# simplerr/rust-renderer

Measured on AMD Instinct MI355X. Metric: Mrays/s (path rays: primary + bounce + sun-shadow + light-shadow) at 1920x1080, 20 spp = 20 frames x 1 spp; camera and sun at rest, the one-off builds of the camera grid and the sun grid outside the timed region (value_with_grid_builds charges them to these frames, value_tree_walk uses neither grid), higher is better.
Workload: dtype f32

## Files before the change

### rust-renderer_amd/csrc/context.hip

```cpp
#include <hip/hip_runtime.h>
#include <rccl/rccl.h>
#include <dlfcn.h>

#include <algorithm>
#include <atomic>
#include <chrono>
#include <cstdlib>
#include <cmath>
#include <cstdio>
#include <cstring>
#include <string>
#include <thread>
#include <vector>

#include "bvh.h"
#include "context_internal.h"
#include "device_scan.h"
#include "device_types.h"
#include "utopian_hip.h"

using namespace uh;

namespace {

std::string g_create_error;

struct HostMesh {
   std::vector<UhVertex> vertices;
   std::vector<uint32_t> indices;
   UhGpuMaterial material;
   float o2w[12];
   float w2o[9];
};

struct EventPair {
   hipEvent_t start, stop;
   int kind;
};

template <typename T>
struct DevBuf {
   T* p = nullptr;
   void* base = nullptr;
   size_t n = 0;
   hipError_t alloc(size_t count, size_t stagger_bytes = 0) {
      release();
      n = count;
      if (count == 0) return hipSuccess;
      hipError_t e = hipMalloc(&base, count * sizeof(T) + stagger_bytes);
      if (e == hipSuccess) p = reinterpret_cast<T*>(static_cast<char*>(base) + stagger_bytes);
      return e;
   }
   void release() {
      if (base) (void)hipFree(base);
      p = nullptr;
      base = nullptr;
      n = 0;
   }
};

struct SceneBins {
   DevBuf<uint32_t> tile_count, tile_cursor, rec_count, tri_mesh, chunks, entries;
   DevBuf<unsigned long long> totals;
   DevBuf<uint4> records;
   DevBuf<float> mats;
   std::vector<float> mats_host;
   uint64_t geom = 0;
   template <class F> void each(F&& f) {
      f(tile_count, 0), f(tile_cursor, 0), f(rec_count, 0), f(tri_mesh, 0), f(chunks, 0), f(entries, 0), f(totals, 0), f(records, 0), f(mats, 0);
   }
};

}

enum HybridStage : int {
   kStShadows, kStGbuffer, kStReflections, kStSsao, kStDeferred, kStSky, kStPresent, kHybridPasses,
   kStEnvCube = kHybridPasses, kStEnvIrradiance, kStEnvSpecular, kStEnvLut, kStShadowMaps, kStMarchingCubes, kHybridStages
};

constexpr uint32_t kMaxSlots = 8;
struct Slot {
   hipStream_t stream = nullptr;
   hipStream_t side = nullptr;
   hipEvent_t ev_traced = nullptr, ev_missed = nullptr, ev_shaded = nullptr, ev_shadowed = nullptr, ev_side_done = nullptr;
   hipEvent_t ev_acc = nullptr;
   hipEvent_t frame_start = nullptr, frame_stop = nullptr;
   DevBuf<float4> rec, radf, pixcol;
   DevBuf<uint32_t> queues[5];
   DevBuf<Control> control;
   PathState ps{};
   bool ready = false;
   size_t capacity = 0;

   hipError_t create(size_t n) {
      capacity = n;
      uint32_t shard_cap = 0;
      {
         const uint32_t runs = (uint32_t)((n + 63) / 64);
         uint32_t per_shard[kShards] = {0};
         for (uint32_t r = 0; r < runs; r++) per_shard[shard_of_run(r)]++;
         for (uint32_t s = 0; s < kShards; s++) shard_cap = per_shard[s] * 64 > shard_cap ? per_shard[s] * 64 : shard_cap;
      }
      hipError_t e;
#define SLOT_TRY(expr)                 \
   if ((e = (expr)) != hipSuccess) return e
      SLOT_TRY(hipStreamCreateWithFlags(&stream, hipStreamNonBlocking));
      SLOT_TRY(hipStreamCreateWithFlags(&side, hipStreamNonBlocking));
      for (hipEvent_t* ev : {&ev_traced, &ev_missed, &ev_shaded, &ev_shadowed, &ev_side_done, &ev_acc}) SLOT_TRY(hipEventCreateWithFlags(ev, hipEventDisableTiming));
      SLOT_TRY(hipEventCreate(&frame_start));
      SLOT_TRY(hipEventCreate(&frame_stop));
      const size_t stagger = 4352;
      const size_t cap_q = (size_t)shard_cap * kShards;
      const size_t plane = (n > cap_q ? n : cap_q) + stagger / sizeof(float4);
      SLOT_TRY(rec.alloc(plane * (2 * kRecQuads + 1), 0 * stagger));
      SLOT_TRY(radf.alloc(n, 1 * stagger));
      SLOT_TRY(pixcol.alloc(n, 2 * stagger));
      for (int qi = 0; qi < 5; qi++) SLOT_TRY(queues[qi].alloc((size_t)shard_cap * kShards * (qi == 4 ? 2 : 1)));
      SLOT_TRY(control.alloc(1));
      SLOT_TRY(hipMemsetAsync(control.p, 0, sizeof(Control), stream));
      SLOT_TRY(hipStreamSynchronize(stream));
#undef SLOT_TRY
      ps.set[0] = PathRecs{rec.p, plane};
      ps.set[1] = PathRecs{rec.p + plane * kRecQuads, plane};
      ps.hit = rec.p + plane * 2 * kRecQuads;
      ps.radf = radf.p;
      ps.pixcol = pixcol.p;
      for (int i = 0; i < 5; i++) ps.queue[i] = queues[i].p;
      ps.shard_cap = shard_cap;
      ready = true;
      return hipSuccess;
   }
   void destroy() {
      if (stream) (void)hipStreamSynchronize(stream);
      if (side) (void)hipStreamSynchronize(side);
      rec.release();
      radf.release();
      pixcol.release();
      for (auto& q : queues) q.release();
      control.release();
      for (hipEvent_t* ev : {&ev_traced, &ev_missed, &ev_shaded, &ev_shadowed, &ev_side_done, &ev_acc, &frame_start, &frame_stop}) {
         if (*ev) (void)hipEventDestroy(*ev);
         *ev = nullptr;
      }
      if (side) (void)hipStreamDestroy(side);
      if (stream) (void)hipStreamDestroy(stream);
      stream = side = nullptr;
      ready = false;
   }
};

constexpr uint32_t kRestirBatch = 16;
constexpr int kSpatialRing = 2 * (int)kRestirBatch + 1;

struct uh_ctx {
   int device = 0;
   Slot slots[kMaxSlots];
   uint32_t frames_in_flight = 4;
   uint32_t batch_frames = 0;
   uint32_t next_slot = 0;
   uint32_t shard_cap = 0;
   hipEvent_t last_acc = nullptr;
   hipStream_t restir_stream = nullptr;
   hipEvent_t ev_restir = nullptr, rs_start = nullptr, rs_stop = nullptr;
   bool restir_recorded = false;
   int spatial_cur = 0;
   hipEvent_t spatial_reader[kSpatialRing] = {};
   uint32_t rp_rank = 0, rp_world = 1, rp_band_rows = 0;
   size_t res_stride = 0;
   UhRestirExchangeFn rp_exchange = nullptr;
   void* rp_user = nullptr;
   hipEvent_t ev_band[kSpatialRing] = {};
   void* rccl = nullptr;
   hipEvent_t t_start = nullptr, t_stop = nullptr;
   Slot* last_slot = nullptr;
   hipStream_t& stream = slots[0].stream;
   PathState& ps = slots[0].ps;
   DevBuf<Control>& control = slots[0].control;
   bool overlap_miss = true, overlap_shadow = true;
   uint32_t W = 0, H = 0;
   uint32_t num_cus = 256;
   uint32_t closest_blocks_per_cu = 5, shadow_blocks_per_cu = 5;
   uint32_t cam_walk_whole = 512;
   bool fused_bounces = true;
   bool fused_always = false;
   static constexpr uint32_t kFusedMaxPaths = 4u << 20;
   uint32_t fused_blocks_per_cu = 4;
   static constexpr uint32_t kSingleFrameBlocksPerCu = 4;
   std::string err;

   std::vector<HostMesh> meshes;
   std::vector<UhGpuLight> lights;
   struct HostTex {
      uint32_t w, h;
      uchar4* dev;
      uint32_t tiles_x;
   };
   std::vector<HostTex> textures;
   bool built = false;

   DevBuf<float4> d_nodes, d_tris, d_shade, d_lights;
   DevBuf<MeshShade> d_meshes;
   DevBuf<float> d_obj_corners, d_world_corners, d_node_box;
   DevBuf<RefitMesh> d_refit_meshes;
   std::vector<uint32_t> packet_keys;
   std::vector<uint32_t> level_start;
   bool topology_valid = false;
   bool device_build = false, src_valid = false;
   uint32_t device_build_kind = 1;
   uint32_t ploc_sah_top = 1024;
   static constexpr uint32_t kPlocRadius = 8;
   DevBuf<float> d_src_corners;
   DevBuf<uint32_t> d_src_keys;
   DevBuf<float4> d_src_shade;
   float refit_ms = 0.0f;
   DevBuf<TexInfo> d_tex;
   DevBuf<float> d_lut;
   SceneDev scene{};

   DevBuf<float4> accumulation, gbuffer;
   DevBuf<uchar4> output;
   DevBuf<UhReservoir> reservoirs[3], spatial_ring;
   DevBuf<float4> gb_ray_o, gb_ray_d, gb_hit;
   DevBuf<DeviceStats> dstats;
   Images im{};

   bool count_visits = false, time_kernels = false, full_frame_restir = false;
   bool iso_reference = true;
   uint32_t shadow_map_size = 4096;
   bool furnace = false;
   uint64_t frames = 0;
   float build_ms = 0.0f, last_frame_ms = 0.0f;
   float ms_by_kind[5] = {0, 0, 0, 0, 0};
   uint32_t trace_closest_launches = 0, trace_light_launches = 0;
   bool frame_timed = false;
   std::vector<EventPair> pending, free_events;
   uint32_t bvh_nodes = 0, bvh_tris = 0;

   bool sun_grid_enabled = true;
   bool sun_valid = false;
   bool sun_attempted = false;
   bool sun_have_pending = false;
   uint64_t geom_version = 1, sun_geom = 0, sun_geom_pending = 0;
   float sun_dir_built[3] = {0, 0, 0}, sun_dir_pending[3] = {0, 0, 0};
   DevBuf<uint32_t> d_sun_cells;
   DevBuf<SunGridEntry> d_sun_entries;
   DevBuf<float4> d_sun_recs;
   DevBuf<float> d_sun_coarse;
   uint32_t sun_coarse_shift = 2;
   int64_t sun_inline_max_mb = -1;
   SunGridDev sun_dev{};
   SunGridLimits sun_limits;
   std::string sun_why;
   float sun_build_ms = 0.0f, sun_mean_list = 0.0f;
   float sun_fallback_area = 1.0f;
   uint32_t sun_cells = 0, sun_entries = 0, sun_max_list = 0;
   bool sun_this_frame = false;
   bool primary_implicit = true;
   bool sun_device_build = true;

   bool cam_grid_enabled = true;
   bool cam_valid = false, cam_attempted = false, cam_have_pending = false;
   uint64_t cam_geom = 0, cam_geom_pending = 0;
   float cam_mats[32] = {0}, cam_mats_pending[32] = {0};
   DevBuf<uint32_t> d_cam_cells;
   DevBuf<SunGridEntry> d_cam_entries;
   SunGridDev cam_dev{};
   SunGridLimits cam_limits;
   std::string cam_why;
   float cam_build_ms = 0.0f, cam_mean_list = 0.0f;
   uint32_t cam_cells = 0, cam_entries = 0, cam_max_list = 0, cam_max_list_interior = 0;
   bool cam_this_frame = false;

   uint32_t tp_rank = 0, tp_world = 1, tp_tile = 64;
   DevBuf<uint32_t> owned_pixels;
   uint32_t n_owned = 0;
   DevBuf<float4> tile_send, tile_recv;
   hipEvent_t ev_compose = nullptr;

   struct Hybrid {
      DevBuf<float4> pos, nrm, pbr;
      DevBuf<uchar4> alb, refl;
      DevBuf<uint8_t> shadow;
      DevBuf<uint32_t> queue, counter;
      DevBuf<HybridMesh> meshes;
      DevBuf<UhVertex> vertices;
      DevBuf<uint32_t> indices;
      uint64_t geom = 0;
      hipEvent_t waits[2 * kMaxSlots + 1] = {};
      struct Stage {
         hipEvent_t begin = nullptr, end = nullptr;
         bool ran = false, timed = false;
         float ms = 0.0f;
      } stage[kHybridStages];
      DevBuf<uint16_t> ssao;
      DevBuf<float4> deferred;
      DevBuf<uchar4> present;
      DevBuf<uint32_t> sky_counter;
      DevBuf<UhGpuLight> raw_lights;
      DevBuf<HybridLight> lights;
      size_t lights_uploaded = SIZE_MAX;
      uint32_t frame_lights = 0;
      DevBuf<float4> env, irr, spec;
      DevBuf<uint32_t> lut;
      DevBuf<float4> taps;
      uint32_t env_builds = 0;
      float env_sun[3] = {0, 0, 0}, env_eye[3] = {0, 0, 0};
      DevBuf<float> smaps;
      DevBuf<uint32_t> s_tile_count, s_tile_cursor, s_rec_count, s_tri_mesh, s_chunks, s_entries;
      DevBuf<unsigned long long> s_totals;
      DevBuf<uint4> s_records;
      DevBuf<float> s_mats;
      DevBuf<UhShadowmapParams> s_params;
      std::vector<float> s_mats_host;
      uint64_t s_geom = 0;
      bool params_set = false;
      UhShadowmapParams params{}, snapshot{}, pending{};
      uint32_t s_renders = 0, smap_size = 0, s_tris[4] = {0, 0, 0, 0};
      bool gbuffer_done = false;
      bool gbuffer_rasterised = false;
      DevBuf<float> gr_depth;
      DevBuf<uint32_t> gr_vis, gr_rec_of, gr_covered;
      SceneBins gr_bins;
      uint32_t gr_renders = 0, gr_pieces = 0;
      DevBuf<float> mc_depth;
      DevBuf<uint32_t> mc_vis, mc_rec_of, mc_covered;
      DevBuf<HybridLight> mc_lights;
      DevBuf<UhVertex> mc_verts;
      DevBuf<uint32_t> mc_block_counts, mc_tile_count, mc_tile_cursor, mc_rec_count, mc_chunks, mc_entries;
      DevBuf<unsigned long long> mc_totals;
      DevBuf<uint4> mc_records;
      DevBuf<float> mc_mats;
      DevBuf<HybridMesh> mc_mesh;
      uint32_t mc_renders = 0, mc_tris = 0, mc_pieces = 0, mc_lights_used = 0;
      float mc_time = 0.0f;

      template <class F> void rt_images(size_t n, F&& f) {
         f(pos, n), f(nrm, n), f(pbr, n), f(alb, n), f(refl, n), f(shadow, n), f(queue, n), f(counter, 1);
      }
      template <class F> void frame_images(size_t n, F&& f) {
         f(ssao, n), f(deferred, n), f(present, n), f(lights, UH_MAX_GPU_LIGHTS + 1), f(sky_counter, 1);
      }
      template <class F> void shadow_maps(F&& f) {
         f(smaps, 0), f(s_tile_count, 0), f(s_tile_cursor, 0), f(s_rec_count, 0), f(s_tri_mesh, 0), f(s_chunks, 0), f(s_entries, 0),
            f(s_totals, 0), f(s_records, 0), f(s_mats, 0), f(s_params, 0);
      }
      template <class F> void mc_images(size_t n, F&& f) {
         f(mc_depth, n), f(mc_vis, n), f(mc_rec_of, n), f(mc_lights, UH_MAX_GPU_LIGHTS + 1), f(mc_block_counts, kMcBlocks), f(mc_mats, 44),
            f(mc_mesh, 1), f(mc_totals, 3), f(mc_covered, 1);
      }
      template <class F> void mc_bins(F&& f) {
         f(mc_verts, 0), f(mc_tile_count, 0), f(mc_tile_cursor, 0), f(mc_rec_count, 0), f(mc_chunks, 0), f(mc_entries, 0), f(mc_records, 0);
      }
      template <class F> void gr_images(size_t n, F&& f) { f(gr_depth, n), f(gr_vis, n), f(gr_rec_of, n), f(gr_covered, 1); }
      template <class F> void env_maps(F&& f) {
         const size_t cube = env_mip_offset(kEnvMips);
         f(env, cube), f(irr, 6 * (size_t)kEnvSize * kEnvSize), f(spec, cube), f(lut, (size_t)kLutSize * kLutSize);
      }
   } hy;

   struct Forward {
      DevBuf<float4> color;
      DevBuf<float> depth;
      DevBuf<uint32_t> vis, rec_of, covered;
      DevBuf<uchar4> present;
      DevBuf<HybridLight> lights;
      SceneBins bins;
      uh_ctx::Hybrid::Stage stage[3];
      uint32_t renders = 0, pieces = 0, lights_used = 0;
      template <class F> void images(size_t n, F&& f) {
         f(depth, n), f(vis, n), f(rec_of, n), f(present, n), f(lights, UH_MAX_GPU_LIGHTS + 1), f(covered, 1), f(color, n);
      }
   } fw;
};

namespace {

int fail(uh_ctx* c, int code, const std::string& msg) {
   if (c)
      c->err = msg;
   else
      g_create_error = msg;
   return code;
}

#define HIP_TRY(ctx, expr)                                                                                   \
   do {                                                                                                      \
      hipError_t e_ = (expr);                                                                                \
      if (e_ != hipSuccess) return fail(ctx, e_ == hipErrorOutOfMemory ? UH_ERR_OUT_OF_MEMORY : UH_ERR_HIP, \
                                        std::string(#expr) + ": " + hipGetErrorString(e_));                 \
   } while (0)

// ... 835 lines not shown
      SunGridDev& d = c->sun_dev;
      std::memcpy(d.U, g.params.U, sizeof(d.U));
      std::memcpy(d.V, g.params.V, sizeof(d.V));
      std::memcpy(d.W, g.params.W, sizeof(d.W));
      d.u0 = g.params.u0;
      d.v0 = g.params.v0;
      d.inv_cell = g.params.inv_cell;
      d.nx = g.params.nx;
      d.ny = g.params.ny;
      d.max_walk = c->sun_limits.max_walk;
      d.cell_start = c->d_sun_cells.p;
      d.entries = c->d_sun_entries.p;
      c->sun_cells = g.params.nx * g.params.ny;
      c->sun_entries = (uint32_t)g.num_entries;
      c->sun_valid = true;
   }
   g.release();
   return attach_sun_inline_records(c);
}

static int attach_sun_inline_records(uh_ctx* c) {
   c->d_sun_recs.release();
   c->sun_dev.recs = nullptr;
   c->d_sun_coarse.release();
   c->sun_dev.coarse = nullptr;
   c->sun_dev.coarse_shift = c->sun_dev.coarse_nx = 0;
   if (c->sun_valid && c->sun_coarse_shift) {
      const uint32_t sh = c->sun_coarse_shift, b = 1u << sh, cnx = (c->sun_dev.nx + b - 1) / b, cny = (c->sun_dev.ny + b - 1) / b;
      HIP_TRY(c, c->d_sun_coarse.alloc((size_t)cnx * cny));
      HIP_TRY(c, (hipError_t)build_sun_coarse_cover((void*)c->stream, c->d_sun_cells.p, c->sun_dev.nx, c->sun_dev.ny, sh, c->d_sun_coarse.p));
      HIP_TRY(c, hipStreamSynchronize(c->stream));
      c->sun_dev.coarse = c->d_sun_coarse.p;
      c->sun_dev.coarse_shift = sh;
      c->sun_dev.coarse_nx = cnx;
   }
   const uint64_t n = c->sun_entries;
   const uint64_t budget = c->sun_inline_max_mb < 0 ? 4ull * 16 * kTriStride16 * c->scene.num_tris : (uint64_t)c->sun_inline_max_mb << 20;
   if (!c->sun_valid || n == 0 || n * 64ull > budget) return UH_OK;
   if (c->d_sun_recs.alloc((size_t)n * 4) != hipSuccess) {
      (void)hipGetLastError();
      return UH_OK;
   }
   HIP_TRY(c, (hipError_t)build_sun_inline_records((void*)c->stream, c->d_tris.p, c->d_sun_entries.p, n, c->d_sun_recs.p));
   HIP_TRY(c, hipStreamSynchronize(c->stream));
   c->sun_dev.recs = reinterpret_cast<const float*>(c->d_sun_recs.p);
   return UH_OK;
}

static int ensure_sun_grid(uh_ctx* c, const float dir[3]) {
   c->sun_this_frame = false;
   if (!c->sun_grid_enabled || c->scene.num_tris == 0) return UH_OK;
   const bool same_geom = c->sun_geom == c->geom_version;
   const bool same_dir = std::memcmp(dir, c->sun_dir_built, sizeof(float) * 3) == 0;
   if (same_geom && c->sun_attempted && same_dir) {
      c->sun_have_pending = false;
      c->sun_this_frame = c->sun_valid;
      return UH_OK;
   }
   if (c->sun_attempted) {
      const bool settled = c->sun_have_pending && c->sun_geom_pending == c->geom_version && std::memcmp(dir, c->sun_dir_pending, sizeof(float) * 3) == 0;
      std::memcpy(c->sun_dir_pending, dir, sizeof(float) * 3);
      c->sun_geom_pending = c->geom_version;
      c->sun_have_pending = true;
      if (!settled) return UH_OK;
   }
   const uint32_t n = c->scene.num_tris;
   if (c->sun_device_build) {
      if (int st = sync_all(c)) return st;
      const auto t0 = std::chrono::steady_clock::now();
      SunGridDevice g;
      const bool ok = build_sun_grid_device((void*)c->stream, c->d_tris.p, n, dir, c->sun_limits, nullptr, g);
      if (!ok && g.why_not.rfind("device build:", 0) == 0) return fail(c, UH_ERR_HIP, "sun grid: " + g.why_not);
      if (int st = adopt_sun_grid_device(c, g, ok, dir, c->geom_version)) return st;
      c->sun_build_ms = std::chrono::duration<float, std::milli>(std::chrono::steady_clock::now() - t0).count();
      c->sun_this_frame = c->sun_valid;
      return UH_OK;
   }
   int threads = (int)std::thread::hardware_concurrency();
   threads = threads < 1 ? 1 : (threads > 32 ? 32 : threads);
   if (int st = sync_all(c)) return st;
   const auto t0 = std::chrono::steady_clock::now();
   std::vector<float> packets(12 * (size_t)n);
   HIP_TRY(c, hipMemcpy2D(packets.data(), sizeof(TriPacket), c->d_tris.p, 16 * kTriStride16, sizeof(TriPacket), n, hipMemcpyDeviceToHost));
   SunGridHost g;
   const bool ok = build_sun_grid(packets.data(), n, dir, c->sun_limits, threads, g);
   if (int st = adopt_sun_grid(c, g, ok, dir, c->geom_version, 0.0f)) return st;
   c->sun_build_ms = std::chrono::duration<float, std::milli>(std::chrono::steady_clock::now() - t0).count();
   c->sun_this_frame = c->sun_valid;
   return UH_OK;
}

static int ensure_camera_grid(uh_ctx* c, const FrameParams& fp, uint32_t batch) {
   c->cam_this_frame = false;
   if (!c->cam_grid_enabled || c->scene.num_tris == 0) return UH_OK;
   float mats[32];
   std::memcpy(mats, fp.inv_view, sizeof(float) * 16);
   std::memcpy(mats + 16, fp.inv_proj, sizeof(float) * 16);
   const bool same = c->cam_attempted && c->cam_geom == c->geom_version && std::memcmp(mats, c->cam_mats, sizeof(mats)) == 0;
   if (same) {
      c->cam_have_pending = false;
      c->cam_this_frame = c->cam_valid;
      return UH_OK;
   }
   const bool settled = c->cam_have_pending && c->cam_geom_pending == c->geom_version && std::memcmp(mats, c->cam_mats_pending, sizeof(mats)) == 0;
   std::memcpy(c->cam_mats_pending, mats, sizeof(mats));
   c->cam_geom_pending = c->geom_version;
   c->cam_have_pending = true;
   if (!settled && batch < 8) return UH_OK;
   if (int st = sync_all(c)) return st;
   const auto t0 = std::chrono::steady_clock::now();
   SunGridDevice g;
   const bool ok = build_camera_grid_device((void*)c->stream, c->d_tris.p, c->scene.num_tris, fp.inv_view, fp.inv_proj, c->W, c->H, c->cam_limits, g);
   if (!ok && g.why_not.rfind("device build:", 0) == 0) return fail(c, UH_ERR_HIP, "camera grid: " + g.why_not);
   c->cam_attempted = true;
   c->cam_have_pending = false;
   c->cam_geom = c->geom_version;
   std::memcpy(c->cam_mats, mats, sizeof(mats));
   c->cam_valid = false;
   c->cam_why = g.why_not;
   c->cam_mean_list = (float)g.mean_list;
   c->cam_max_list = g.max_list;
   c->cam_max_list_interior = g.max_list_interior;
   c->cam_cells = c->cam_entries = 0;
   c->d_cam_cells.release();
   c->d_cam_entries.release();
   if (ok) {
      const size_t ncell = (size_t)g.params.nx * g.params.ny;
      c->d_cam_cells.p = g.cells;
      c->d_cam_cells.base = g.cells;
      c->d_cam_cells.n = ncell + 1;
      c->d_cam_entries.p = g.entries;
      c->d_cam_entries.base = g.entries;
      c->d_cam_entries.n = (size_t)g.num_entries;
      g.cells = nullptr;
      g.entries = nullptr;
      SunGridDev& d = c->cam_dev;
      d = SunGridDev{};
      d.nx = g.params.nx;
      d.ny = g.params.ny;
      d.max_walk = c->cam_limits.max_walk;
      d.walk_whole = c->cam_walk_whole;
      d.cell_start = c->d_cam_cells.p;
      d.entries = c->d_cam_entries.p;
      c->cam_cells = c->W * c->H;
      c->cam_entries = (uint32_t)g.num_entries;
      c->cam_valid = true;
   }
   g.release();
   c->cam_build_ms = std::chrono::duration<float, std::milli>(std::chrono::steady_clock::now() - t0).count();
   c->cam_this_frame = c->cam_valid;
   return UH_OK;
}

static int enqueue_path_trace(uh_ctx* c, Slot& s, const FrameParams& fp) {
   LaunchCfg lc = cfg(c);
   lc.stream = s.stream;
   if (fp.batch_frames == 1) {
      lc.closest_blocks_per_cu = std::min(lc.closest_blocks_per_cu, uh_ctx::kSingleFrameBlocksPerCu);
      lc.shadow_blocks_per_cu = std::min(lc.shadow_blocks_per_cu, uh_ctx::kSingleFrameBlocksPerCu);
   }
   Control* ctl = s.control.p;
   DeviceStats* st = c->dstats.p;
   for (uint32_t smp = 0; smp < fp.samples_per_frame; smp++) {
      HIP_TRY(c, hipMemsetAsync(ctl, 0, sizeof(Control), s.stream));
      uint32_t slot = 0;
      launch_generate(lc, fp, s.ps, ctl, smp);
      const bool gpu_idle = !c->last_acc || hipEventQuery(c->last_acc) == hipSuccess;
      const bool fused = c->fused_bounces && fp.batch_frames == 1 && fp.num_bounces >= 2 && fp.num_bounces <= 64 && s.ps.shard_cap < (1u << 23) &&
                         ((gpu_idle && fp.n_owned <= uh_ctx::kFusedMaxPaths) || c->fused_always);
      const bool fused_sun0 = fused && fp.sun_shadow_enabled == 1 && fp.lights_enabled != 1;
      for (uint32_t b = 0; b < (fused ? 1u : fp.num_bounces); b++) {
         begin_timed(c, (b == 0 && c->cam_this_frame) ? 3 : 0, s.stream);
         if (b == 0 && c->cam_this_frame) {
            launch_trace_camera_grid(lc, fp, c->scene, s.ps, ctl, st, slot, slot + 1, c->cam_dev, c->cam_max_list_interior > std::max(c->cam_dev.walk_whole, c->cam_dev.max_walk));
            slot += 2;
         } else
            launch_trace_closest(lc, c->scene, s.ps, ctl, st, b, slot++, b == 0 ? UH_RAY_PRIMARY : UH_RAY_BOUNCE);
         end_timed(c, s.stream);
         const bool side_shadow = c->overlap_shadow && (fp.sun_shadow_enabled == 1 || fp.lights_enabled == 1);
         const bool side_used = side_shadow || c->overlap_miss;
         if (side_used && b > 0) HIP_TRY(c, hipStreamWaitEvent(s.stream, s.ev_shadowed, 0));
         begin_timed(c, 2, s.stream);
         launch_shade_hit(lc, fp, c->scene, s.ps, c->im, ctl, st, b);
         if (!c->overlap_miss) launch_shade_miss(lc, fp, s.ps, ctl, st, b);
         end_timed(c, s.stream);
         LaunchCfg lsh = lc;
         hipStream_t sh_stream = s.stream;
         if (side_used) {
            HIP_TRY(c, hipEventRecord(s.ev_shaded, s.stream));
            HIP_TRY(c, hipStreamWaitEvent(s.side, s.ev_shaded, 0));
         }
         if (c->overlap_miss) {
            LaunchCfg ls = lc;
            ls.stream = s.side;
            begin_timed(c, 2, s.side);
            launch_shade_miss(ls, fp, s.ps, ctl, st, b);
            end_timed(c, s.side);
         }
         if (side_shadow) {
            lsh.stream = s.side;
            sh_stream = s.side;
         }
         if (fp.sun_shadow_enabled == 1 && !fused_sun0) {
            begin_timed(c, 1, sh_stream);
            if (c->sun_this_frame) {
               launch_trace_sun_grid(lsh, fp, c->scene, s.ps, ctl, st, b, slot++, c->sun_dev);
               launch_trace_shadow(lsh, fp, c->scene, s.ps, ctl, st, b, slot++, false, true);
            } else
               launch_trace_shadow(lsh, fp, c->scene, s.ps, ctl, st, b, slot++, false);
            end_timed(c, sh_stream);
         }
         if (fp.lights_enabled == 1) {
            begin_timed(c, 4, sh_stream);
            launch_trace_shadow(lsh, fp, c->scene, s.ps, ctl, st, b, slot++, true);
            end_timed(c, sh_stream);
         }
         if (side_used) HIP_TRY(c, hipEventRecord(s.ev_shadowed, s.side));
      }
      const bool join_side = (c->overlap_miss || c->overlap_shadow) && fp.num_bounces > 0;
      if (join_side && !fused_sun0) {
         HIP_TRY(c, hipEventRecord(s.ev_side_done, s.side));
         HIP_TRY(c, hipStreamWaitEvent(s.stream, s.ev_side_done, 0));
      }
      if (fused) {
         begin_timed(c, 0, s.stream);
         launch_path_fused(lc, fp, c->scene, s.ps, ctl, st, c->sun_dev, c->sun_this_frame, fused_sun0);
         end_timed(c, s.stream);
      }
      if (join_side && fused_sun0) {
         HIP_TRY(c, hipEventRecord(s.ev_side_done, s.side));
         HIP_TRY(c, hipStreamWaitEvent(s.stream, s.ev_side_done, 0));
      }
      if (fp.num_bounces > 0 && !fused) launch_flush_survivors(lc, fp, s.ps, ctl);
      const bool last = smp + 1 == fp.samples_per_frame;
      if (last && c->last_acc && c->last_acc != s.ev_acc) HIP_TRY(c, hipStreamWaitEvent(s.stream, c->last_acc, 0));
      launch_finish_sample(lc, fp, s.ps, c->im, smp, last);
   }
   if (fp.samples_per_frame == 0) {
      if (c->last_acc && c->last_acc != s.ev_acc) HIP_TRY(c, hipStreamWaitEvent(s.stream, c->last_acc, 0));
      launch_resolve(lc, c->im, c->W, c->H, fp.total_samples, fp.accumulation_limit);
   }
   HIP_TRY(c, hipEventRecord(s.ev_acc, s.stream));
   c->last_acc = s.ev_acc;
   return UH_OK;
}

struct uh_batch {
   FrameParams fp;
   uint32_t pass_mask = 0, batch = 0;
   bool restir_frame = false, reads_reservoirs = false;
   int read_slot[kMaxBatchFrames];
   LaunchCfg rc;
};

static UhReservoir* spatial_buf(uh_ctx* c, int slot) { return slot ? c->spatial_ring.p + (size_t)(slot - 1) * c->res_stride : c->reservoirs[2].p; }

static void restir_rows(const uh_ctx* c, UhRestirRows& r) {
   const uint32_t H = c->H, B = c->rp_world > 1 ? c->rp_band_rows : H;
   r = UhRestirRows{};
   r.rows_per_band = B;
   const uint32_t b0 = std::min<uint64_t>((uint64_t)c->rp_rank * B, H), b1 = std::min<uint64_t>((uint64_t)b0 + B, H);
   r.band_row0 = b0;
   r.band_rows = b1 - b0;
   if (b1 == b0) return;
   const uint32_t halo = 30;
   const uint32_t t0 = b0 > halo ? b0 - halo : 0, t1 = std::min<uint64_t>((uint64_t)b1 + halo, H);
   r.reuse_row0 = t0;
   r.reuse_rows = t1 - t0;
   if (b0 < halo && t1 < H) {
      r.reuse_extra_row0 = H - 1;
      r.reuse_extra_rows = 1;
   }
   const uint32_t g0 = t0 > 0 ? t0 - 1 : 0;
   r.cast_row0 = g0;
   r.cast_rows = t1 - g0;
   if (r.reuse_extra_rows) {
      const uint32_t e0 = std::max(H >= 2 ? H - 2 : 0u, t1);
      r.cast_extra_row0 = e0;
      r.cast_extra_rows = H - e0;
   }
}
static RowSpans spans_of(const uh_ctx* c, uint32_t row0, uint32_t rows, uint32_t extra0, uint32_t extra_rows) { return RowSpans{{row0, extra0}, {rows, extra_rows}, c->W}; }

static int batch_begin(uh_ctx* c, const UhViewUniformData* view, uint32_t pass_mask, uint32_t batch, uh_batch& bs) {
   if (!c) return UH_ERR_INVALID_ARGUMENT;
   if (!view) return fail(c, UH_ERR_INVALID_ARGUMENT, "uh_render_frame: null view");
   if (!c->built && c->topology_valid && view->rebuild_tlas == 1) {
      if (int st = uh_refit_acceleration(c)) return st;
   }
   if (!c->built) return fail(c, UH_ERR_NOT_BUILT, "uh_render_frame before uh_build_acceleration");
   if (view->num_bounces > kMaxBounces) return fail(c, UH_ERR_INVALID_ARGUMENT, "num_bounces > 64");
   if (view->samples_per_frame > 4096) return fail(c, UH_ERR_INVALID_ARGUMENT, "samples_per_frame > 4096 (the reference UI stops at 10)");
   if (view->num_lights > c->lights.size() && (view->lights_enabled == 1 || (pass_mask & UH_PASS_RESTIR)))
      return fail(c, UH_ERR_INVALID_ARGUMENT, "view.num_lights exceeds the lights added with uh_add_light");
   HIP_TRY(c, hipSetDevice(c->device));
   FrameParams& fp = bs.fp;
   fp = make_params(c, *view);
   fp.batch_frames = batch;
   for (uint32_t f = 0; f < batch; f++) {
      const uint32_t total = view->total_samples + f * view->samples_per_frame;
      fp.total_samples_of[f] = total;
      fp.frame_numbers[f] = (uint32_t)(int32_t)((float)total + view->time * 10000.0f);
   }
   c->cam_this_frame = false;
   const bool primary_rays = ((pass_mask & UH_PASS_REFERENCE_PT) && fp.num_bounces > 0 && fp.samples_per_frame > 0) || (pass_mask & UH_PASS_GBUFFER);
   if (primary_rays)
      if (int st = ensure_camera_grid(c, fp, batch)) return st;
   fp.primary_implicit = (c->primary_implicit && c->cam_this_frame && fp.samples_per_frame == 1) ? 1u : 0u;
   bs.pass_mask = pass_mask;
   bs.batch = batch;
   bs.restir_frame = (pass_mask & UH_PASS_RESTIR) != 0;
   bs.reads_reservoirs = (pass_mask & UH_PASS_REFERENCE_PT) && fp.lights_enabled == 1 && fp.use_ris == 1;

   if (batch > 1 && !(pass_mask & UH_PASS_REFERENCE_PT)) return fail(c, UH_ERR_INVALID_ARGUMENT, "uh_render_frames: a batch needs the path-tracing pass");
   if (batch > kRestirBatch && bs.restir_frame) return fail(c, UH_ERR_INVALID_ARGUMENT, "uh_render_frames: more reservoir-pass frames in one batch than the spatial ring holds");
   c->t_start = c->t_stop = nullptr;
   for (uint32_t f = 0; f < kMaxBatchFrames; f++) bs.read_slot[f] = c->spatial_cur;

   if (bs.restir_frame) {
      if (!c->restir_stream) {
         HIP_TRY(c, hipStreamCreateWithFlags(&c->restir_stream, hipStreamNonBlocking));
         HIP_TRY(c, hipEventCreateWithFlags(&c->ev_restir, hipEventDisableTiming));
         HIP_TRY(c, hipEventCreate(&c->rs_start));
// ... 292 lines not shown
      }
   }
   d_o.release();
   dd.release();
   dh.release();
   return UH_OK;
}

int uh_trace_any(uh_ctx* c, const float* rays, uint32_t n, uint8_t* out_occluded) {
   if (!c) return UH_ERR_INVALID_ARGUMENT;
   if (!c->built) return fail(c, UH_ERR_NOT_BUILT, "uh_trace_any before uh_build_acceleration");
   if (n == 0) return UH_OK;
   if (!rays || !out_occluded) return fail(c, UH_ERR_INVALID_ARGUMENT, "null argument");
   HIP_TRY(c, hipSetDevice(c->device));
   std::vector<float4> o(n), d(n);
   for (uint32_t i = 0; i < n; i++) {
      const float* r = rays + 8 * (size_t)i;
      o[i] = make_float4(r[0], r[1], r[2], r[3]);
      d[i] = make_float4(r[4], r[5], r[6], r[7]);
   }
   DevBuf<float4> d_o, dd;
   DevBuf<uint32_t> occ;
   HIP_TRY(c, d_o.alloc(n));
   HIP_TRY(c, dd.alloc(n));
   HIP_TRY(c, occ.alloc(n));
   HIP_TRY(c, hipMemcpyAsync(d_o.p, o.data(), n * sizeof(float4), hipMemcpyHostToDevice, c->stream));
   HIP_TRY(c, hipMemcpyAsync(dd.p, d.data(), n * sizeof(float4), hipMemcpyHostToDevice, c->stream));
   begin_timed(c, 1);
   launch_trace_any_raw(cfg(c), c->scene, d_o.p, dd.p, occ.p, n);
   end_timed(c);
   std::vector<uint32_t> h(n);
   if (int st = staged_read(c, h.data(), occ.p, n * sizeof(uint32_t))) return st;
   for (uint32_t i = 0; i < n; i++) out_occluded[i] = h[i] ? 1 : 0;
   d_o.release();
   dd.release();
   occ.release();
   return UH_OK;
}

int uh_get_stats(uh_ctx* c, UhStats* out) {
   if (!c || !out) return UH_ERR_INVALID_ARGUMENT;
   HIP_TRY(c, hipSetDevice(c->device));
   if (int st = sync_all(c)) return st;
   DeviceStats ds;
   if (int st = staged_read(c, &ds, c->dstats.p, sizeof(ds))) return st;
   drain_timed(c);
   if (c->frame_timed) {
      float ms = 0.0f;
      if (c->t_start && c->t_stop && hipEventElapsedTime(&ms, c->t_start, c->t_stop) == hipSuccess) c->last_frame_ms = ms;
   }
   std::memset(out, 0, sizeof(*out));
   for (int i = 0; i < UH_RAY_KINDS; i++) out->rays[i] = ds.rays[i];
   out->nodes_visited = ds.nodes_visited;
   out->tris_tested = ds.tris_tested;
   out->shadow_nodes_visited = ds.shadow_nodes_visited;
   out->shadow_tris_tested = ds.shadow_tris_tested;
   out->closest_hits = ds.closest_hits;
   out->misses = ds.misses;
   out->frames = c->frames;
   out->bvh_nodes = c->bvh_nodes;
   out->bvh_triangles = c->bvh_tris;
   out->build_ms = c->build_ms;
   out->last_frame_ms = c->last_frame_ms;
   out->trace_closest_ms = c->ms_by_kind[0];
   out->trace_shadow_ms = c->ms_by_kind[1];
   out->shade_ms = c->ms_by_kind[2];
   out->camera_grid_ms = c->ms_by_kind[3];
   out->trace_light_ms = c->ms_by_kind[4];
   out->trace_light_launches = c->trace_light_launches;
   out->light_nodes_visited = ds.light_nodes_visited;
   out->light_tris_tested = ds.light_tris_tested;
   out->trace_closest_launches = c->trace_closest_launches;
   out->sun_grid_cells = c->sun_valid ? c->sun_cells : 0;
   out->sun_grid_entries = c->sun_valid ? c->sun_entries : 0;
   out->sun_grid_build_ms = c->sun_build_ms;
   out->sun_grid_mean_list = c->sun_mean_list;
   out->sun_tree_rays = ds.sun_tree_rays;
   out->camera_grid_cells = c->cam_valid && c->cam_this_frame ? c->cam_cells : 0;
   out->camera_grid_entries = c->cam_valid && c->cam_this_frame ? c->cam_entries : 0;
   out->camera_grid_build_ms = c->cam_build_ms;
   out->camera_grid_mean_list = c->cam_mean_list;
   out->camera_tree_rays = ds.cam_tree_rays;
   out->camera_grid_tris_tested = ds.cam_tris_tested;
   out->sun_covered_rays = ds.sun_covered_rays;
   if (c->sun_valid) out->sun_grid_bytes = c->d_sun_cells.n * sizeof(uint32_t) + c->d_sun_entries.n * sizeof(SunGridEntry) + c->d_sun_recs.n * sizeof(float4) + c->d_sun_coarse.n * sizeof(float);
   if (c->cam_valid && c->cam_this_frame) out->camera_grid_bytes = c->d_cam_cells.n * sizeof(uint32_t) + c->d_cam_entries.n * sizeof(SunGridEntry);
   return UH_OK;
}

int uh_reset_stats(uh_ctx* c) {
   if (!c) return UH_ERR_INVALID_ARGUMENT;
   HIP_TRY(c, hipSetDevice(c->device));
   if (int st = sync_all(c)) return st;
   drain_timed(c);
   HIP_TRY(c, hipMemsetAsync(c->dstats.p, 0, sizeof(DeviceStats), c->stream));
   HIP_TRY(c, hipStreamSynchronize(c->stream));
   c->frames = 0;
   for (float& ms : c->ms_by_kind) ms = 0.0f;
   c->trace_closest_launches = c->trace_light_launches = 0;
   return UH_OK;
}

int uh_set_option(uh_ctx* c, const char* name, int value) {
   if (!c) return UH_ERR_INVALID_ARGUMENT;
   if (!name) return fail(c, UH_ERR_INVALID_ARGUMENT, "null option name");
   const std::string n(name);
   auto range = [&](int lo, int hi) { return value >= lo && value <= hi; };
   auto bad = [&](const char* what) { return fail(c, UH_ERR_INVALID_ARGUMENT, n + " " + what); };
   if (n == "count_visits")
      c->count_visits = value != 0;
   else if (n == "time_kernels") {
      if (c->time_kernels && !value) {
         (void)sync_all(c);
         drain_timed(c);
      }
      c->time_kernels = value != 0;
   }
   else if (n == "device_build") {
      if (!range(0, 2)) return bad("must be 0, 1 (PLOC) or 2 (radix tree)");
      if (c->device_build != (value != 0) || (value && c->device_build_kind != (uint32_t)value)) c->built = c->topology_valid = false;
      c->device_build = value != 0;
      if (value) c->device_build_kind = (uint32_t)value;
   } else if (n == "ploc_sah_top") {
      if (!range(0, 1 << 20)) return bad("must be 0..1048576");
      if (c->ploc_sah_top != (uint32_t)value && c->device_build) c->built = c->topology_valid = false;
      c->ploc_sah_top = (uint32_t)value;
   }
   else if (n == "sun_grid")
      c->sun_grid_enabled = value != 0;
   else if (n == "sun_grid_build") {
      c->sun_device_build = value != 0;
      c->sun_attempted = false;
   } else if (n == "sun_grid_density") {
      if (!range(1, 4096)) return bad("(entries per triangle) must be 1..4096");
      c->sun_limits.entries_per_triangle = (double)value;
      c->sun_attempted = false;
   } else if (n == "sun_grid_max_walk") {
      if (!range(1, 4096)) return bad("(longest list a ray tests itself) must be 1..4096");
      c->sun_limits.max_walk = (uint32_t)value;
      c->sun_attempted = false;
   } else if (n == "sun_grid_max_mb") {
      if (!range(1, 65536)) return bad("must be 1..65536");
      c->sun_limits.max_entries = ((uint64_t)value << 20) / sizeof(SunGridEntry);
      c->sun_attempted = false;
   } else if (n == "sun_grid_force") {
      const SunGridLimits defaults;
      c->sun_limits.max_mean_list = value ? 1e30 : defaults.max_mean_list;
      c->sun_limits.max_fallback_area = value ? 2.0 : defaults.max_fallback_area;
      c->sun_attempted = false;
   } else if (n == "sun_grid_inline_max_mb") {
      if (!range(-1, 1 << 20)) return bad("must be -1 (auto: 4 x the packet array), 0 (off) .. 1048576");
      c->sun_inline_max_mb = value;
      c->sun_attempted = false;
   } else if (n == "sun_grid_coarse") {
      if (!range(0, 6)) return bad("(log2 of the block edge in cells) must be 0..6");
      c->sun_coarse_shift = (uint32_t)value;
      c->sun_attempted = false;
   }
   else if (n == "camera_grid")
      c->cam_grid_enabled = value != 0;
   else if (n == "camera_grid_max_walk") {
      if (!range(1, 4096)) return bad("must be 1..4096");
      c->cam_limits.max_walk = (uint32_t)value;
      c->cam_attempted = false;
   } else if (n == "camera_grid_walk_whole") {
      if (!range(0, 65536)) return bad("must be 0..65536");
      c->cam_walk_whole = (uint32_t)value;
      c->cam_attempted = false;
   } else if (n == "camera_grid_max_mean_list_x10") {
      if (!range(1, 100000)) return bad("must be 1..100000");
      c->cam_limits.max_mean_list = value / 10.0;
      c->cam_attempted = false;
   } else if (n == "primary_implicit")
      c->primary_implicit = value != 0;
   else if (n == "full_frame_restir")
      c->full_frame_restir = value != 0;
   else if (n == "iso_reference_triangulation")
      c->iso_reference = value != 0;
   else if (n == "furnace")
      c->furnace = value != 0;
   else if (n == "shadow_map_size") {
      if (!range(16, 8192)) return bad("must be 16..8192");
      if ((uint32_t)value != c->shadow_map_size) {
         if (int st = sync_all(c)) return st;
         c->hy.shadow_maps([](auto& b, size_t) { b.release(); });
         c->hy.s_geom = 0;
         c->hy.smap_size = 0;
      }
      c->shadow_map_size = (uint32_t)value;
   }
   else if (n == "overlap")
      c->overlap_miss = c->overlap_shadow = value != 0;
   else if (n == "batch_frames") {
      if (!range(0, (int)kMaxBatchFrames)) return bad("must be 0 (auto) .. 32");
      c->batch_frames = (uint32_t)value;
   } else if (n == "frames_in_flight") {
      if (!range(1, (int)kMaxSlots)) return bad("must be 1..8");
      (void)sync_all(c);
      c->frames_in_flight = (uint32_t)value;
      c->next_slot = 0;
   } else if (n == "fused_bounces") {
      if (!range(-1, 8)) return bad("must be 0 (off), 1 (on when no frame is in flight), -1 (always on) or 2..8 (as 1, and blocks per CU of its grid)");
      c->fused_bounces = value != 0;
      c->fused_always = value == -1;
      if (value >= 2) c->fused_blocks_per_cu = (uint32_t)value;
   } else if (n == "trace_blocks_per_cu") {
      if (!range(1, 8)) return bad("must be 1..8");
      c->closest_blocks_per_cu = c->shadow_blocks_per_cu = (uint32_t)value;
   } else
      return fail(c, UH_ERR_INVALID_ARGUMENT, "unknown option: " + n);
   return UH_OK;
}

int uh_set_tile_partition(uh_ctx* c, uint32_t rank, uint32_t world, uint32_t tile_size) {
   if (!c) return UH_ERR_INVALID_ARGUMENT;
   if (world == 0 || rank >= world || tile_size == 0) return fail(c, UH_ERR_INVALID_ARGUMENT, "uh_set_tile_partition: need rank < world, tile_size > 0");
   HIP_TRY(c, hipSetDevice(c->device));
   if (int st = sync_all(c)) return st;
   c->tp_rank = rank;
   c->tp_world = world;
   c->tp_tile = tile_size;
   c->n_owned = c->W * c->H;
   c->owned_pixels.release();
   if (world > 1) {
      const uint32_t tiles_x = (c->W + tile_size - 1) / tile_size;
      std::vector<uint32_t> own;
      own.reserve((size_t)c->W * c->H / world + 1);
      for (uint32_t y = 0; y < c->H; y++)
         for (uint32_t x = 0; x < c->W; x++)
            if (((y / tile_size) * tiles_x + x / tile_size) % world == rank) own.push_back(y * c->W + x);
      c->n_owned = (uint32_t)own.size();
      HIP_TRY(c, c->owned_pixels.alloc(own.size() ? own.size() : 1));
      if (!own.empty()) HIP_TRY(c, hipMemcpy(c->owned_pixels.p, own.data(), own.size() * 4, hipMemcpyHostToDevice));
   }
   return UH_OK;
}

int uh_set_restir_partition(uh_ctx* c, uint32_t rank, uint32_t world, UhRestirExchangeFn exchange, void* user) {
   if (!c) return UH_ERR_INVALID_ARGUMENT;
   if (world == 0 || rank >= world) return fail(c, UH_ERR_INVALID_ARGUMENT, "uh_set_restir_partition: need rank < world");
   HIP_TRY(c, hipSetDevice(c->device));
   if (int st = sync_all(c)) return st;
   const size_t npix = (size_t)c->W * c->H;
   const uint32_t band_rows = (c->H + world - 1) / world;
   const size_t stride = std::max(npix, (size_t)band_rows * world * c->W);
   if (stride != c->res_stride) {
      DevBuf<UhReservoir> fresh;
      HIP_TRY(c, fresh.alloc(stride));
      HIP_TRY(c, hipMemsetAsync(fresh.p, 0, stride * sizeof(UhReservoir), c->stream));
      HIP_TRY(c, hipMemcpyAsync(fresh.p, c->im.reservoirs[2], npix * sizeof(UhReservoir), hipMemcpyDeviceToDevice, c->stream));
      HIP_TRY(c, hipStreamSynchronize(c->stream));
      c->reservoirs[2].release();
      c->reservoirs[2] = fresh;
      fresh.p = nullptr;
      fresh.n = 0;
      c->spatial_ring.release();
      c->res_stride = stride;
   } else if (c->spatial_cur != 0) {
      HIP_TRY(c, hipMemcpyAsync(c->reservoirs[2].p, c->im.reservoirs[2], npix * sizeof(UhReservoir), hipMemcpyDeviceToDevice, c->stream));
      HIP_TRY(c, hipStreamSynchronize(c->stream));
   }
   c->spatial_cur = 0;
   for (auto& r : c->spatial_reader) r = nullptr;
   c->im.reservoirs[2] = c->reservoirs[2].p;
   c->im.prev_spatial = c->reservoirs[2].p;
   c->rp_rank = rank;
   c->rp_world = world;
   c->rp_band_rows = world > 1 ? band_rows : c->H;
   c->rp_exchange = exchange;
   c->rp_user = user;
   return UH_OK;
}

int uh_get_restir_rows(uh_ctx* c, UhRestirRows* out) {
   if (!c || !out) return UH_ERR_INVALID_ARGUMENT;
   restir_rows(c, *out);
   return UH_OK;
}

namespace {
struct RcclApi {
   void* so = nullptr;
   decltype(&ncclGetUniqueId) GetUniqueId = nullptr;
   decltype(&ncclCommInitRank) CommInitRank = nullptr;
   decltype(&ncclCommDestroy) CommDestroy = nullptr;
   decltype(&ncclAllGather) AllGather = nullptr;
   decltype(&ncclSend) Send = nullptr;
   decltype(&ncclRecv) Recv = nullptr;
   decltype(&ncclGroupStart) GroupStart = nullptr;
   decltype(&ncclGroupEnd) GroupEnd = nullptr;
   decltype(&ncclCommCount) CommCount = nullptr;
   decltype(&ncclGetErrorString) GetErrorString = nullptr;
   std::string why;
};
RcclApi* rccl_api() {
   static RcclApi api;
   static bool tried = false;
   if (tried) return &api;
   tried = true;
   for (const char* name : {"librccl.so.1", "librccl.so", "/opt/rocm/lib/librccl.so.1"}) {
      api.so = dlopen(name, RTLD_NOW | RTLD_GLOBAL);
      if (api.so) break;
   }
   if (!api.so) {
      api.why = std::string("librccl not found: ") + (dlerror() ? dlerror() : "");
      return &api;
   }
// ... 1290 lines not shown
```

### rust-renderer_amd/csrc/device_types.h

```cpp
#pragma once
#include <hip/hip_runtime.h>

#include <cstdint>
#include <vector>

#include "bvh.h"
#include "sun_grid.h"
#include "utopian_hip.h"

namespace uh {

constexpr uint32_t kMaxBounces = 64;
constexpr uint32_t kQueueKinds = 5;
enum { Q_RAY = 0, Q_LIGHT = 1, Q_SUN_TREE = 2, Q_MISS = 3, Q_CAM_TREE = 4 };
constexpr uint32_t kLaunchSlots = kMaxBounces * 4 + 8;

constexpr uint32_t kShards = 32;
constexpr uint32_t kShardBits = 5;
static_assert((1u << kShardBits) == kShards, "kShards is a power of two");
__host__ __device__ inline uint32_t shard_of_run(uint32_t run) { return (run * 0x9E3779B1u) >> (32 - kShardBits); }

constexpr uint32_t kBounceStride = ((kMaxBounces + 1 + 31) / 32) * 32;
constexpr uint32_t kSlotStride = ((kLaunchSlots + 31) / 32) * 32;
struct Control {
   uint32_t q_count[kShards * kQueueKinds * kBounceStride];
   uint32_t cursor[kShards * kSlotStride];
};
__host__ __device__ inline uint32_t qc_index(uint32_t bounce, uint32_t kind, uint32_t shard) { return (shard * kQueueKinds + kind) * kBounceStride + bounce; }
__host__ __device__ inline uint32_t cursor_index(uint32_t slot, uint32_t shard) { return shard * kSlotStride + slot; }

struct DeviceStats {
   unsigned long long rays[UH_RAY_KINDS];
   unsigned long long nodes_visited, tris_tested, shadow_nodes_visited, shadow_tris_tested;
   unsigned long long closest_hits, misses;
   unsigned long long sun_tree_rays;
   unsigned long long cam_tree_rays;
   unsigned long long cam_tris_tested;
   unsigned long long sun_covered_rays;
   unsigned long long light_nodes_visited, light_tris_tested;
};

struct alignas(16) MeshShade {
   float w2o[9];
   uint32_t diffuse_map;
   float base_color[3];
   float type;
   float property;
   uint32_t pad;
   float metallic, roughness;
   float pad2[2];
};
static_assert(sizeof(MeshShade) == 80, "mesh shading record");

struct TexInfo {
   const uchar4* texels;
   uint32_t w, h;
   uint32_t tiles_x;
   uint32_t pad;
};

struct SceneDev {
   const uint4* nodes;
   const float4* tris;
   const float4* shade;
   const MeshShade* meshes;
   const TexInfo* textures;
   const float4* lights;
   const float* unorm_lut;
   uint32_t num_nodes, num_tris, num_meshes, num_textures, num_lights;
};

constexpr uint32_t kMaxBatchFrames = 32;

struct FrameParams {
   uint32_t batch_frames;
   uint32_t frame_numbers[kMaxBatchFrames];
   uint32_t total_samples_of[kMaxBatchFrames];
   const UhReservoir* spatial_of[kMaxBatchFrames];
   float inv_view[16], inv_proj[16], prev_pv[16];
   float sun_dir[3];
   uint32_t W, H, frame_number;
   uint32_t samples_per_frame, total_samples, num_bounces, accumulation_limit;
   uint32_t sky_enabled, sun_shadow_enabled, lights_enabled, use_ris, full_frame_restir;
   uint32_t primary_implicit;
   uint32_t furnace;
   uint32_t num_lights_used;
   uint32_t temporal_enabled, spatial_enabled;
   uint32_t tp_rank, tp_world, tp_tile, tiles_x;
   const uint32_t* owned_pixels;
   uint32_t n_owned;
};

constexpr uint32_t kRecQuads = 4;
enum { REC_ORIGIN = 0, REC_DIR = 1, REC_THR = 2, REC_RAD = 3 };
struct PathRecs {
   float4* base;
   size_t plane;
};
struct PathState {
   PathRecs set[2];
   float4* hit;
   float4* radf;
   float4* pixcol;
   uint32_t* queue[5];
   uint32_t shard_cap;
};
__host__ __device__ inline float4* rec_quad(const PathRecs& rec, uint32_t pos, int quad) { return rec.base + rec.plane * (size_t)quad + pos; }

struct RawRays {
   float4* ray_o;
   float4* ray_d;
   float4* hit;
};

struct Images {
   float4* accumulation;
   uchar4* output;
   float4* gbuffer_pos;
   UhReservoir* reservoirs[3];
   const UhReservoir* prev_spatial;
};

struct RowSpans {
   uint32_t row0[2], rows[2];
   uint32_t W;
   __host__ __device__ uint32_t total() const { return (rows[0] + rows[1]) * W; }
   __host__ __device__ uint32_t pixel_of(uint32_t j) const {
      const uint32_t first = rows[0] * W;
      return j < first ? row0[0] * W + j : row0[1] * W + (j - first);
   }
};
inline RowSpans whole_frame(uint32_t W, uint32_t H) { return RowSpans{{0, 0}, {H, 0}, W}; }

struct HybridMesh {
   float o2w[9];
   float w2o[9];
   uint32_t vertex_base, index_base;
   uint32_t diffuse_map, normal_map, metallic_roughness_map, occlusion_map;
};
struct HybridDev {
   float4* pos;
   float4* nrm;
   uchar4* alb;
   float4* pbr;
   uint8_t* shadow;
   uchar4* refl;
   uint32_t* queue;
   uint32_t* counter;
   const HybridMesh* meshes;
   const UhVertex* vertices;
   const uint32_t* indices;
   float sun_dir[3];
   float eye[3];
   uint32_t W, H, furnace;
};
struct HybridLight {
   float pos[3];
   float mode;
   float color[3];
   float spot;
   float att[3];
   float pad0;
   float dir[3];
   float pad1;
};
struct HybridFrameDev {
   uint16_t* ssao;
   float4* deferred;
   uchar4* present;
   uint32_t* sky_counter;
   HybridLight* lights;
   const UhGpuLight* raw_lights;
   float view[16], proj[16], inv_view[16];
   uint32_t num_lights;
   uint32_t ssao_on, rt_on, fxaa_on;
   float sun_raw[3];
};

struct LaunchCfg {
   hipStream_t stream;
   uint32_t num_cus;
   uint32_t closest_blocks_per_cu, shadow_blocks_per_cu;
   bool count_visits;
   uint32_t fused_blocks_per_cu = 4;
};

void launch_generate(const LaunchCfg&, const FrameParams&, const PathState&, Control*, uint32_t sample);
void launch_trace_closest(const LaunchCfg&, const SceneDev&, const PathState&, Control*, DeviceStats*, uint32_t bounce, uint32_t cursor_slot,
                          int ray_kind);
void launch_trace_camera_grid(const LaunchCfg&, const FrameParams&, const SceneDev&, const PathState&, Control*, DeviceStats*, uint32_t cursor_slot_grid, uint32_t cursor_slot_tree,
                              const SunGridDev&, bool leftovers_possible = true);
void launch_shade_miss(const LaunchCfg&, const FrameParams&, const PathState&, Control*, DeviceStats*, uint32_t bounce);
void launch_shade_hit(const LaunchCfg&, const FrameParams&, const SceneDev&, const PathState&, const Images&, Control*, DeviceStats*, uint32_t bounce);
void launch_flush_survivors(const LaunchCfg&, const FrameParams&, const PathState&, Control*);
void launch_path_fused(const LaunchCfg&, const FrameParams&, const SceneDev&, const PathState&, Control*, DeviceStats*, const SunGridDev& g, bool use_grid, bool sun_of_bounce0);
void launch_trace_shadow(const LaunchCfg&, const FrameParams&, const SceneDev&, const PathState&, Control*, DeviceStats*, uint32_t bounce,
                         uint32_t cursor_slot, bool light, bool sun_leftovers = false);
void launch_trace_sun_grid(const LaunchCfg&, const FrameParams&, const SceneDev&, const PathState&, Control*, DeviceStats*, uint32_t bounce,
                           uint32_t cursor_slot, const SunGridDev&);
void launch_finish_sample(const LaunchCfg&, const FrameParams&, const PathState&, const Images&, uint32_t sample, bool last);
void launch_resolve(const LaunchCfg&, const Images&, uint32_t W, uint32_t H, uint32_t total_samples, uint32_t limit);
void launch_gbuffer(const LaunchCfg&, const FrameParams&, const SceneDev&, const RawRays&, const Images&, DeviceStats*, const RowSpans& spans, uint32_t counted,
                    const SunGridDev* camera_grid = nullptr);
void launch_reset_reservoirs(const LaunchCfg&, const FrameParams&, const Images&, const RowSpans& spans);
void launch_initial_ris(const LaunchCfg&, const FrameParams&, const SceneDev&, const Images&, const RowSpans& spans);
void launch_temporal_reuse(const LaunchCfg&, const FrameParams&, const SceneDev&, const Images&, const RowSpans& spans);
void launch_spatial_reuse(const LaunchCfg&, const FrameParams&, const SceneDev&, const Images&, const RowSpans& spans);
void launch_trace_closest_raw(const LaunchCfg&, const SceneDev&, const float4* ray_o, const float4* ray_d, float4* hit, uint32_t n);
void launch_trace_any_raw(const LaunchCfg&, const SceneDev&, const float4* ray_o, const float4* ray_d, uint32_t* occluded, uint32_t n);
void launch_hybrid_clear(const LaunchCfg&, const HybridDev&);
void launch_hybrid_gbuffer(const LaunchCfg&, const FrameParams&, const SceneDev&, const HybridDev&, const SunGridDev* camera_grid);
void launch_hybrid_shadows(const LaunchCfg&, const SceneDev&, const HybridDev&);
void launch_hybrid_frame_clear(const LaunchCfg&, const HybridDev&, const HybridFrameDev&);
void launch_hybrid_ssao(const LaunchCfg&, const HybridDev&, const HybridFrameDev&);
void launch_hybrid_present(const LaunchCfg&, const HybridDev&, const HybridFrameDev&);
constexpr uint32_t kEnvSize = 512, kEnvMips = 8, kLutSize = 512;
constexpr uint32_t kIrrPhi = 252, kIrrTheta = 63;
__host__ __device__ inline uint32_t env_mip_offset(uint32_t m) {
   uint32_t o = 0;
   for (uint32_t k = 0; k < m; k++) o += 6u * (kEnvSize >> k) * (kEnvSize >> k);
   return o;
}
struct IblMaps {
   const float4* env;
   const float4* irr;
   const float4* spec;
   const uint32_t* lut;
};
struct EnvDev {
   float4* env;
   float4* irr;
   float4* spec;
   uint32_t* lut;
   const float4* taps;
   float eye[3];
   float sun[3];
};
void launch_env_cube(const LaunchCfg&, const EnvDev&);
void launch_env_irradiance(const LaunchCfg&, const EnvDev&);
void launch_env_specular(const LaunchCfg&, const EnvDev&);
void launch_env_brdf_lut(const LaunchCfg&, const EnvDev&);
void launch_hybrid_reflections(const LaunchCfg&, const SceneDev&, const HybridDev&, const IblMaps* ibl);
struct ShadowLookup {
   const float* maps;
   const UhShadowmapParams* params;
   uint32_t size;
};
void launch_hybrid_deferred(const LaunchCfg&, const SceneDev&, const HybridDev&, const HybridFrameDev&, const IblMaps* ibl,
                            const ShadowLookup* shadow);
constexpr uint32_t kShadowTile = 128;
struct ShadowDev {
   const UhVertex* vertices;
   const uint32_t* indices;
   const HybridMesh* meshes;
   const uint32_t* tri_mesh;
   const float* mats;
   uint32_t num_tris, num_meshes, size, tiles_x;
// ... 88 lines not shown
```

### rust-renderer_amd/csrc/kernels.hip

```cpp
#include <hip/hip_runtime.h>

#include <type_traits>

#include "device_math.h"
#include "device_types.h"
#include "hybrid_shading.h"
#include "ibl_device.h"

namespace uh {

constexpr int kBlock = 256;
constexpr int kWavesPerBlock = kBlock / 64;
constexpr int kSunRaysPerLane = 2;
constexpr int kShadeHitBlocks = 4;
constexpr int kLdsStack = 16;
constexpr int kSpillStack = (int)kTraversalStackEntries - kLdsStack;

struct Hit {
   float t, u, v;
   uint32_t idx;
   uint32_t key;
};

__device__ __forceinline__ float dot_fma(V3 a, V3 b) { return fmaf(a.z, b.z, fmaf(a.y, b.y, a.x * b.x)); }
// ... 257 lines not shown
         n = load_n;
         pool_base = load_base;
         loading = false;
      }
   }

   template <typename SrcFn>
   __device__ __forceinline__ void advance(const RaySource& src, RayPool<NA>& pool, SrcFn&& source_of) {
      const uint32_t lane = lane_id();
      if (q_n) {
         asm volatile("s_waitcnt lgkmcnt(0)" ::: "memory");
         if (lane < q_n) {
#pragma unroll
            for (int a = 0; a < NA; a++) dma16(source_of(a, q_id), pool.v[a]);
            pool.id[lane] = q_id;
         }
         load_n = q_n;
         load_base = q_base;
         loading = true;
         q_n = 0;
      }
      if (have_base) {
         const uint32_t b = __builtin_amdgcn_readfirstlane(r_base);
         have_base = false;
         if (b < src.count) {
            q_base = b;
            q_n = src.count - b < kPool ? src.count - b : kPool;
            if (lane < q_n) q_id = src.queue ? ld_stream(src.queue + b + lane) : b + lane;
         } else {
            drained = true;
         }
      }
      if (!drained) {
         if (src.cursor) {
            if (lane == 0) r_base = atomicAdd(src.cursor, kPool);
         } else {
            r_base = (static_k * src.num_waves + src.wave_index) * kPool;
            static_k++;
         }
         have_base = true;
      }
   }
};

constexpr int kRefill = 8;
template <int NA, typename SrcFn, typename TakeFn>
__device__ __forceinline__ bool refill_lanes(Feeder<NA>& f, const RaySource& src, RayPool<NA>& pool, bool lane_idle, SrcFn&& source_of, TakeFn&& take) {
   if (++f.iterations > (1u << 24)) return false;
   const unsigned long long idle = __ballot(lane_idle);
   if (idle == 0ull) return true;
   const uint32_t n_idle = (uint32_t)__popcll(idle);
   f.land();
   const uint32_t avail = f.n - f.pos;
   if (avail != 0 && (n_idle >= (uint32_t)kRefill || n_idle == 64u)) {
      const uint32_t prefix = __builtin_amdgcn_mbcnt_hi((uint32_t)(idle >> 32), __builtin_amdgcn_mbcnt_lo((uint32_t)idle, 0u));
      if (lane_idle && prefix < avail) take(f.pos + prefix);
      f.pos += n_idle < avail ? n_idle : avail;
   }
   if (f.pos >= f.n && !f.loading) {
      if (f.empty()) return n_idle != 64u || avail != 0;
      f.advance(src, pool, source_of);
   }
   return true;
}

template <bool ANY, bool COUNT, bool CAP = false>
__device__ __forceinline__ bool trav_step(const uint4* __restrict__ nodes, const float4* __restrict__ tris, Trav& t, uint32_t* lds_col, uint32_t* spill, bool& occluded,
                                          uint32_t& n_nodes, uint32_t& n_tris) {
   const bool at_node = !(t.cur & kLeafBit);
   const uint32_t packet = t.cur & ~kLeafBit;
   const uint4* rec = at_node ? nodes + kNodeStride16 * (size_t)packet : (const uint4*)tris + kTriStride16 * (size_t)packet;
   uint4 w0 = rec[0], w1 = rec[1], w2 = rec[2];
   asm volatile("" : "+v"(w2.z), "+v"(w2.w));
   bool pop;
   if (at_node) {
      if (COUNT) n_nodes++;
      pop = !node_compute<ANY, CAP>(w0, w1, w2, t, lds_col, spill);
   } else {
      if (COUNT) n_tris++;
      const float4 ta = make_float4(__uint_as_float(w0.x), __uint_as_float(w0.y), __uint_as_float(w0.z), __uint_as_float(w0.w));
      const float4 tb = make_float4(__uint_as_float(w1.x), __uint_as_float(w1.y), __uint_as_float(w1.z), __uint_as_float(w1.w));
      const float4 tc = make_float4(__uint_as_float(w2.x), __uint_as_float(w2.y), __uint_as_float(w2.z), __uint_as_float(w2.w));
      pop = true;
      if (tri_compute<ANY>(ta, tb, tc, packet, t.o, t.d, t.tmin, t.tlimit, t.best) && ANY) {
         occluded = true;
         t.cur = kEmptyRef;
         pop = false;
      }
   }
   if (pop) t.cur = trav_pop(t, lds_col, spill);
   return t.cur == kEmptyRef;
}

template <bool COUNT>
__global__ __launch_bounds__(kBlock, 6) void k_trace_closest(SceneDev sc, bool sharded, const float4* __restrict__ ray_o,
                                                               const float4* __restrict__ ray_d, float4* __restrict__ hit_out, uint32_t shard_cap, Control* ctl,
                                                               DeviceStats* stats, uint32_t bounce, uint32_t cursor_slot, int ray_kind, uint32_t raw_count,
                                                               const uint32_t* __restrict__ listed) {
   const bool range_in_w = !sharded;
   __shared__ uint32_t s_stack[kWavesPerBlock][kLdsStack][64];
   __shared__ RayPool<2> s_pool[kWavesPerBlock];
   const uint32_t lane = lane_id();
   const uint32_t wave = threadIdx.x >> 6;
   uint32_t* lds_col = &s_stack[wave][0][lane];
   RayPool<2>& pool = s_pool[wave];
   RaySource src;
   uint32_t seg = 0;
   if (sharded) {
      const ShardCtx sx = shard_ctx();
      seg = sx.shard * shard_cap;
      src.queue = listed ? listed + seg : nullptr;
      src.count = ctl->q_count[qc_index(bounce, listed ? Q_CAM_TREE : Q_RAY, sx.shard)];
      src.cursor = &ctl->cursor[cursor_index(cursor_slot, sx.shard)];
      src.wave_index = src.num_waves = 0;
      if (sx.lb == 0 && threadIdx.x == 0) {
         if (!listed) atomicAdd(&stats->rays[ray_kind], (unsigned long long)src.count);
         else if (src.count) atomicAdd(&stats->cam_tree_rays, (unsigned long long)src.count);
      }
   } else {
      src.queue = nullptr;
      src.count = raw_count;
      src.cursor = nullptr;
      src.wave_index = blockIdx.x * kWavesPerBlock + wave;
      src.num_waves = gridDim.x * kWavesPerBlock;
   }
   const uint4* __restrict__ nodes = sc.nodes;
   const float4* __restrict__ tris = sc.tris;
   auto source_of = [&](int a, uint32_t pos) { return (a == 0 ? ray_o : ray_d) + seg + pos; };
   Feeder<2> f;
   Trav t;
   t.cur = kEmptyRef;
   t.sp = 0;
   uint32_t where = 0, n_nodes = 0, n_tris = 0;
   uint32_t spill[kSpillStack];
   auto take = [&](uint32_t slot) {
      where = seg + (listed ? pool.id[slot] : f.pool_base + slot);
      const float4 ro = pool.v[0][slot], rd = pool.v[1][slot];
      trav_init(t, ro, rd, range_in_w ? ro.w : 0.001f, range_in_w ? rd.w : 10000.0f, INFINITY);
   };
   while (refill_lanes<2>(f, src, pool, t.cur == kEmptyRef, source_of, take)) {
      if (t.cur != kEmptyRef) {
         bool occluded = false;
         if (trav_step<false, COUNT>(nodes, tris, t, lds_col, spill, occluded, n_nodes, n_tris))
            st_rec(hit_out + where, make_float4(t.best.t, t.best.u, t.best.v, __uint_as_float(t.best.idx)));
      }
   }
   if (COUNT) {
      atomicAdd(&stats->nodes_visited, (unsigned long long)n_nodes);
      atomicAdd(&stats->tris_tested, (unsigned long long)n_tris);
   }
}

struct ShadowRay {
   float4 ro, rd, lit;
   float tlimit;
};
template <bool LIGHT>
__device__ __forceinline__ ShadowRay make_shadow_ray(const SceneDev& sc, const FrameParams& fp, float4 ro, float4 thr, float4 rad) {
   ShadowRay s;
   s.ro = make_float4(ro.x, ro.y, ro.z, 0.001f);
   s.tlimit = INFINITY;
   if (LIGHT) {
      const int light_index = (int)__float_as_uint(rad.w);
      V3 lpos = v3(0, 0, 0);
      if (light_index >= 0 && (uint32_t)light_index < sc.num_lights) lpos = xyz(sc.lights[2 * light_index]);
      const V3 o = v3(ro.x, ro.y, ro.z);
      const V3 dir = normalize3(lpos - o);
      s.tlimit = length3(lpos - o);
      const float f = thr.w;
      s.lit = make_float4(rad.x + thr.x * f, rad.y + thr.y * f, rad.z + thr.z * f, rad.w);
      s.rd = make_float4(dir.x, dir.y, dir.z, 10000.0f);
   } else {
      s.lit = make_float4(rad.x + thr.x, rad.y + thr.y, rad.z + thr.z, rad.w);
      s.rd = make_float4(fp.sun_dir[0], fp.sun_dir[1], fp.sun_dir[2], 10000.0f);
   }
   return s;
}

template <bool COUNT, bool LIGHT>
__global__ __launch_bounds__(kBlock, 5) void k_trace_shadow(SceneDev sc, FrameParams fp, PathState ps, Control* ctl, DeviceStats* stats, uint32_t bounce,
                                                              uint32_t cursor_slot, bool leftovers) {
   __shared__ uint32_t s_stack[kWavesPerBlock][kLdsStack][64];
   __shared__ RayPool<3> s_pool[kWavesPerBlock];
   const uint32_t lane = lane_id();
   const uint32_t wave = threadIdx.x >> 6;
   uint32_t* lds_col = &s_stack[wave][0][lane];
   RayPool<3>& pool = s_pool[wave];
   const ShardCtx sx = shard_ctx();
   const uint32_t seg = sx.shard * ps.shard_cap;
   RaySource src;
   src.queue = LIGHT ? ps.queue[2] + seg : leftovers ? ps.queue[3] + seg : nullptr;
   src.count = LIGHT ? ctl->q_count[qc_index(bounce, Q_LIGHT, sx.shard)] : leftovers ? ctl->q_count[qc_index(bounce, Q_SUN_TREE, sx.shard)] : ctl->q_count[qc_index(bounce + 1, Q_RAY, sx.shard)];
   src.cursor = &ctl->cursor[cursor_index(cursor_slot, sx.shard)];
   src.wave_index = src.num_waves = 0;
   if (sx.lb == 0 && threadIdx.x == 0) {
      if (!leftovers) atomicAdd(&stats->rays[LIGHT ? UH_RAY_LIGHT_SHADOW : UH_RAY_SUN_SHADOW], (unsigned long long)src.count);
      else if (src.count) atomicAdd(&stats->sun_tree_rays, (unsigned long long)src.count);
   }
   const uint4* __restrict__ nodes = sc.nodes;
   const float4* __restrict__ tris = sc.tris;
   const PathRecs rec = ps.set[(bounce + 1) & 1];
   float4* rad = rec_quad(rec, seg, REC_RAD);
   auto source_of = [&](int a, uint32_t pos) { return (const float4*)rec_quad(rec, seg + pos, a == 0 ? REC_ORIGIN : a == 1 ? REC_THR : REC_RAD); };
   Feeder<3> f;
   Trav t;
   t.cur = kEmptyRef;
   t.sp = 0;
   uint32_t id = 0, n_nodes = 0, n_tris = 0;
   float4 lit = make_float4(0.0f, 0.0f, 0.0f, 0.0f);
   uint32_t spill[kSpillStack];
   auto take = [&](uint32_t slot) {
      id = pool.id[slot];
      const ShadowRay s = make_shadow_ray<LIGHT>(sc, fp, pool.v[0][slot], pool.v[1][slot], pool.v[2][slot]);
      lit = s.lit;
      trav_init(t, s.ro, s.rd, s.ro.w, s.rd.w, s.tlimit);
   };
   while (refill_lanes<3>(f, src, pool, t.cur == kEmptyRef, source_of, take)) {
      if (t.cur != kEmptyRef) {
         bool occluded = false;
         if (trav_step<true, COUNT>(nodes, tris, t, lds_col, spill, occluded, n_nodes, n_tris) && !occluded) st_stream(rad + id, lit);
      }
   }
   if (COUNT) {
      atomicAdd(LIGHT ? &stats->light_nodes_visited : &stats->shadow_nodes_visited, (unsigned long long)n_nodes);
      atomicAdd(LIGHT ? &stats->light_tris_tested : &stats->shadow_tris_tested, (unsigned long long)n_tris);
   }
}

template <int N, int I = 0, typename F>
__device__ __forceinline__ void static_for(F&& f) {
   if constexpr (I < N) {
      f(std::integral_constant<int, I>{});
      static_for<N, I + 1>(f);
   }
}

__device__ __forceinline__ void sun_cell_of(const SunGridDev& g, float pu, float pv, uint32_t& cx, uint32_t& cy) {
   float fx = (pu - g.u0) * g.inv_cell, fy = (pv - g.v0) * g.inv_cell;
   fx = !(fx >= 0.0f) ? 0.0f : fx;
   fy = !(fy >= 0.0f) ? 0.0f : fy;
   const float max_x = (float)(g.nx - 1), max_y = (float)(g.ny - 1);
   fx = fx > max_x ? max_x : fx;
   fy = fy > max_y ? max_y : fy;
   cx = (uint32_t)fx;
   cy = (uint32_t)fy;
}
__device__ __forceinline__ bool sun_coarse_covered(float coarse, float pw) { return pw < coarse && coarse - pw < kSunCoarseReach; }

template <bool COUNT, bool INLINE>
__global__ __launch_bounds__(kBlock) void k_trace_sun_grid(SceneDev sc, FrameParams fp, PathState ps, Control* ctl, DeviceStats* stats, uint32_t bounce,
                                                            uint32_t cursor_slot, SunGridDev g) {
   const uint32_t lane = lane_id();
   const ShardCtx sx = shard_ctx();
   const uint32_t seg = sx.shard * ps.shard_cap;
   const PathRecs rec = ps.set[(bounce + 1) & 1];
   const uint32_t count = ctl->q_count[qc_index(bounce + 1, Q_RAY, sx.shard)];
   uint32_t* cursor = &ctl->cursor[cursor_index(cursor_slot, sx.shard)];
   const V3 d = v3(fp.sun_dir[0], fp.sun_dir[1], fp.sun_dir[2]);
   uint32_t n_tris = 0, n_covered = 0;
   uint32_t* q_tree = ps.queue[3] + seg;
   uint32_t* n_tree = &ctl->q_count[qc_index(bounce, Q_SUN_TREE, sx.shard)];
   constexpr int K = kSunRaysPerLane;
   typedef float f4_t __attribute__((ext_vector_type(4)));
   const f4_t* __restrict__ recs = reinterpret_cast<const f4_t*>(g.recs);
   const f4_t* __restrict__ tris = reinterpret_cast<const f4_t*>(sc.tris);
   const uint2* __restrict__ entries = reinterpret_cast<const uint2*>(g.entries);
   const uint4* __restrict__ cells = reinterpret_cast<const uint4*>(g.cell_start);
   for (;;) {
      uint32_t base = 0;
      if (lane == 0) base = atomicAdd(cursor, 64u * K);
      base = __builtin_amdgcn_readfirstlane(base);
      if (base >= count) break;
      uint32_t id[K];
      bool valid[K];
      static_for<K>([&](auto kc) {
         constexpr int k = decltype(kc)::value;
         id[k] = base + 64u * k + lane;
         valid[k] = id[k] < count;
      });
      float4 ro[K];
      static_for<K>([&](auto kc) {
         constexpr int k = decltype(kc)::value;
         ro[k] = valid[k] ? ld_rec(rec_quad(rec, seg + id[k], REC_ORIGIN)) : make_float4(0.0f, 0.0f, 0.0f, 0.0f);
      });
      float pw[K];
      uint32_t cx[K], cy[K];
      bool covered[K], ask[K];
      static_for<K>([&](auto kc) {
         constexpr int k = decltype(kc)::value;
         const V3 o = v3(ro[k].x, ro[k].y, ro[k].z);
         const float pu = dot_fma(v3(g.U[0], g.U[1], g.U[2]), o), pv = dot_fma(v3(g.V[0], g.V[1], g.V[2]), o);
         pw[k] = dot_fma(v3(g.W[0], g.W[1], g.W[2]), o);
         sun_cell_of(g, pu, pv, cx[k], cy[k]);
         covered[k] = false;
      });
      if (g.coarse) {
         float cw[K];
         static_for<K>([&](auto kc) {
            constexpr int k = decltype(kc)::value;
            cw[k] = valid[k] ? g.coarse[(cy[k] >> g.coarse_shift) * g.coarse_nx + (cx[k] >> g.coarse_shift)] : -INFINITY;
         });
         static_for<K>([&](auto kc) {
            constexpr int k = decltype(kc)::value;
            covered[k] = valid[k] && sun_coarse_covered(cw[k], pw[k]);
         });
      }
      uint4 cs[K];
      uint32_t end[K];
      static_for<K>([&](auto kc) {
         constexpr int k = decltype(kc)::value;
         ask[k] = valid[k] && !covered[k];
         cs[k] = make_uint4(0u, 0u, 0u, 0u);
         end[k] = 0u;
         if (ask[k]) {
            const uint32_t cell = cy[k] * g.nx + cx[k];
            cs[k] = cells[cell];
            end[k] = cells[cell + 1].x;
         }
      });
      bool defer[K], walk[K], lit[K];
      f4_t ra[K], rb[K], rc[K];
      uint2 en[K], nxt[K];
      static_for<K>([&](auto kc) {
         constexpr int k = decltype(kc)::value;
         const float cover = __uint_as_float(cs[k].y);
         const bool cov = ask[k] && pw[k] < cover && cover - pw[k] < kSunCoverReach;
         covered[k] = covered[k] || cov;
         defer[k] = ask[k] && !cov && (cx[k] == 0 || cy[k] == 0 || cx[k] + 1 == g.nx || cy[k] + 1 == g.ny || end[k] - cs[k].x > g.max_walk);
         walk[k] = ask[k] && !cov && !defer[k] && cs[k].x < end[k];
         lit[k] = ask[k] && !cov && !defer[k] && !walk[k];
         if (walk[k]) {
            if constexpr (INLINE) {
               const f4_t* r = recs + 4 * (size_t)cs[k].x;
               ra[k] = r[0];
               rb[k] = r[1];
               rc[k] = r[2];
            } else {
               en[k] = make_uint2(cs[k].z, cs[k].w);
               if (__uint_as_float(en[k].y) < pw[k]) {
                  walk[k] = false;
                  lit[k] = true;
               } else {
                  const f4_t* r = tris + kTriStride16 * (size_t)en[k].x;
                  ra[k] = r[0];
                  rb[k] = r[1];
                  rc[k] = r[2];
                  nxt[k] = cs[k].x + 1 < end[k] ? entries[cs[k].x + 1] : make_uint2(0u, 0u);
               }
            }
         }
         if (COUNT) n_covered += covered[k] ? 1u : 0u;
      });
      static_for<K>([&](auto kc) {
         constexpr int k = decltype(kc)::value;
         if (walk[k]) {
            const V3 o = v3(ro[k].x, ro[k].y, ro[k].z);
            Hit best;
            best.t = 10000.0f;
            best.u = best.v = 0.0f;
            best.idx = kEmptyRef;
            best.key = 0xffffffffu;
            uint32_t e = cs[k].x;
            float4 a = make_float4(ra[k].x, ra[k].y, ra[k].z, ra[k].w), b = make_float4(rb[k].x, rb[k].y, rb[k].z, rb[k].w), c = make_float4(rc[k].x, rc[k].y, rc[k].z, rc[k].w);
            bool occluded = false;
            if constexpr (INLINE) {
               const f4_t* r = recs + 4 * (size_t)e;
               for (;;) {
                  if (c.z < pw[k]) break;
                  if (COUNT) n_tris++;
                  if (tri_compute<true>(a, b, c, 0u, o, d, 0.001f, INFINITY, best)) {
                     occluded = true;
                     break;
                  }
                  e++;
                  if (e >= end[k] || c.w < pw[k]) break;
                  r += 4;
                  const f4_t na = r[0], nb = r[1], nc = r[2];
                  a = make_float4(na.x, na.y, na.z, na.w);
                  b = make_float4(nb.x, nb.y, nb.z, nb.w);
                  c = make_float4(nc.x, nc.y, nc.z, nc.w);
               }
            } else {
               uint2 cur = en[k], nx = nxt[k];
               for (;;) {
                  if (COUNT) n_tris++;
                  if (tri_compute<true>(a, b, c, cur.x, o, d, 0.001f, INFINITY, best)) {
                     occluded = true;
                     break;
                  }
                  e++;
                  if (e >= end[k] || __uint_as_float(nx.y) < pw[k]) break;
                  cur = nx;
                  if (e + 1 < end[k]) nx = entries[e + 1];
                  const f4_t* r = tris + kTriStride16 * (size_t)cur.x;
                  const f4_t na = r[0], nb = r[1], nc = r[2];
                  a = make_float4(na.x, na.y, na.z, na.w);
                  b = make_float4(nb.x, nb.y, nb.z, nb.w);
                  c = make_float4(nc.x, nc.y, nc.z, nc.w);
               }
            }
            lit[k] = !occluded;
         }
      });
      float4 thr[K], rad[K];
      static_for<K>([&](auto kc) {
         constexpr int k = decltype(kc)::value;
         if (lit[k]) {
            thr[k] = ld_rec(rec_quad(rec, seg + id[k], REC_THR));
            rad[k] = ld_rec(rec_quad(rec, seg + id[k], REC_RAD));
         }
      });
      static_for<K>([&](auto kc) {
         constexpr int k = decltype(kc)::value;
         if (lit[k]) st_rec(rec_quad(rec, seg + id[k], REC_RAD), make_float4(rad[k].x + thr[k].x, rad[k].y + thr[k].y, rad[k].z + thr[k].z, rad[k].w));
      });
      static_for<K>([&](auto kc) {
         constexpr int k = decltype(kc)::value;
         if (__ballot(defer[k]) != 0ull) {
            const uint32_t slot = wave_append(n_tree, defer[k]);
            if (defer[k]) st_stream(q_tree + slot, id[k]);
         }
      });
   }
   if (sx.lb == 0 && threadIdx.x == 0) {
      atomicAdd(&stats->rays[UH_RAY_SUN_SHADOW], (unsigned long long)count);
      if (COUNT) atomicAdd(&stats->shadow_nodes_visited, (unsigned long long)count);
   }
   if (COUNT) {
      atomicAdd(&stats->shadow_tris_tested, (unsigned long long)n_tris);
      atomicAdd(&stats->sun_covered_rays, (unsigned long long)n_covered);
   }
}

template <bool COUNT>
__global__ __launch_bounds__(kBlock) void k_trace_camera_grid(SceneDev sc, FrameParams fp, PathState ps, Control* ctl, DeviceStats* stats, uint32_t cursor_slot, SunGridDev g) {
   const uint32_t lane = lane_id();
   const ShardCtx sx = shard_ctx();
   const uint32_t seg = sx.shard * ps.shard_cap;
   const uint32_t* __restrict__ queue = ps.queue[0] + seg;
   const uint32_t count = ctl->q_count[qc_index(0, Q_RAY, sx.shard)];
   uint32_t* cursor = &ctl->cursor[cursor_index(cursor_slot, sx.shard)];
   const PathRecs rec = ps.set[0];
   const float4* __restrict__ tris = sc.tris;
   uint32_t* q_tree = ps.queue[3] + seg;
   uint32_t* n_tree = &ctl->q_count[qc_index(0, Q_CAM_TREE, sx.shard)];
   uint32_t n_tris = 0;
   for (;;) {
      const uint32_t base = next_batch(cursor);
      if (base >= count) break;
      const uint32_t i = base + lane;
      const bool valid = i < count;
      bool defer = false;
      if (valid) {
         const uint32_t id = ld_stream(queue + i);
         const uint32_t k = id % fp.n_owned;
         const uint32_t pix = fp.owned_pixels ? fp.owned_pixels[k] : k;
         const uint32_t px = pix % fp.W, py = pix / fp.W;
         const uint32_t cell = (py + 1) * g.nx + (px + 1);
         uint32_t e = g.cell_start[cell];
         const uint32_t end = g.cell_start[cell + 1];
         const bool sorted = end - e <= g.max_walk;
         defer = end - e > (g.walk_whole > g.max_walk ? g.walk_whole : g.max_walk);
         if (defer && fp.primary_implicit) {
            float4 ro, rd;
            primary_state(fp, id, ro, rd);
            st_rec(rec_quad(rec, seg + i, REC_ORIGIN), ro);
            st_rec(rec_quad(rec, seg + i, REC_DIR), rd);
         }
         if (!defer) {
            float4 ro, rd;
            if (fp.primary_implicit)
               primary_state(fp, id, ro, rd);
            else {
               ro = ld_rec(rec_quad(rec, seg + i, REC_ORIGIN));
               rd = ld_rec(rec_quad(rec, seg + i, REC_DIR));
            }
            const V3 o = v3(ro.x, ro.y, ro.z), d = v3(rd.x, rd.y, rd.z);
            Hit best;
            best.t = 10000.0f;
            best.u = best.v = 0.0f;
            best.idx = kEmptyRef;
            best.key = 0xffffffffu;
            uint2 en = make_uint2(0u, 0u);
            if (e < end) en = reinterpret_cast<const uint2*>(g.entries)[e];
            while (e < end) {
               if (sorted && -__uint_as_float(en.y) > best.t) break;
               const uint32_t pk = en.x;
               uint2 nxt = make_uint2(0u, 0u);
               if (e + 1 < end) nxt = reinterpret_cast<const uint2*>(g.entries)[e + 1];
               const float4 a = tris[kTriStride16 * (size_t)pk + 0], b = tris[kTriStride16 * (size_t)pk + 1], c = tris[kTriStride16 * (size_t)pk + 2];
               if (COUNT) n_tris++;
               tri_compute<false>(a, b, c, pk, o, d, 0.001f, INFINITY, best);
               en = nxt;
               e++;
            }
            st_rec(ps.hit + seg + i, make_float4(best.t, best.u, best.v, __uint_as_float(best.idx)));
         }
      }
      if (__ballot(defer) != 0ull) {
         const uint32_t slot = wave_append(n_tree, defer);
         if (defer) st_stream(q_tree + slot, i);
      }
   }
   if (sx.lb == 0 && threadIdx.x == 0) atomicAdd(&stats->rays[UH_RAY_PRIMARY], (unsigned long long)count);
   if (COUNT) atomicAdd(&stats->cam_tris_tested, (unsigned long long)n_tris);
}

__global__ __launch_bounds__(kBlock) void k_gbuffer_camera_grid(SceneDev sc, RawRays ps, RowSpans spans, uint32_t W, SunGridDev g) {
   const uint32_t n = spans.total();
   const float4* __restrict__ tris = sc.tris;
   for (uint32_t j = blockIdx.x * kBlock + threadIdx.x; j < n; j += gridDim.x * kBlock) {
      const uint32_t pix = spans.pixel_of(j);
      const uint32_t px = pix % W, py = pix / W;
      const uint32_t cell = (py + 1) * g.nx + (px + 1);
      uint32_t e = g.cell_start[cell];
      const uint32_t end = g.cell_start[cell + 1];
      const bool sorted = end - e <= g.max_walk;
      const float4 ro = ps.ray_o[j], rd = ps.ray_d[j];
      const V3 o = v3(ro.x, ro.y, ro.z), d = v3(rd.x, rd.y, rd.z);
      Hit best;
      best.t = rd.w;
      best.u = best.v = 0.0f;
      best.idx = kEmptyRef;
      best.key = 0xffffffffu;
      for (; e < end; e++) {
         const uint2 en = reinterpret_cast<const uint2*>(g.entries)[e];
         if (sorted && -__uint_as_float(en.y) > best.t) break;
         const uint32_t pk = en.x;
         const float4 a = tris[kTriStride16 * (size_t)pk + 0], b = tris[kTriStride16 * (size_t)pk + 1], c = tris[kTriStride16 * (size_t)pk + 2];
         tri_compute<false>(a, b, c, pk, o, d, ro.w, INFINITY, best);
      }
      ps.hit[j] = make_float4(best.t, best.u, best.v, __uint_as_float(best.idx));
   }
}

__global__ __launch_bounds__(kBlock) void k_trace_any_raw(SceneDev sc, const float4* __restrict__ ray_o, const float4* __restrict__ ray_d,
                                                          uint32_t* __restrict__ occluded, uint32_t count) {
   __shared__ uint32_t s_stack[kWavesPerBlock][kLdsStack][64];
   uint32_t* lds_col = &s_stack[threadIdx.x >> 6][0][lane_id()];
   uint32_t n_nodes = 0, n_tris = 0;
   for (uint32_t i = blockIdx.x * kBlock + threadIdx.x; i < count; i += gridDim.x * kBlock) {
      float4 ro = ray_o[i], rd = ray_d[i];
      Hit h;
      occluded[i] = traverse<true, false>(sc, v3(ro.x, ro.y, ro.z), v3(rd.x, rd.y, rd.z), ro.w, rd.w, INFINITY, h, lds_col, n_nodes, n_tris) ? 1u : 0u;
   }
}

__global__ __launch_bounds__(kBlock) void k_generate(FrameParams fp, PathState ps, Control* ctl, uint32_t sample) {
   const uint32_t n = fp.n_owned * fp.batch_frames;
   const uint32_t lane = lane_id();
   const uint32_t groups = (n + 63) / 64;
   for (uint32_t g = blockIdx.x * kWavesPerBlock + (threadIdx.x >> 6); g < groups; g += gridDim.x * kWavesPerBlock) {
      const uint32_t q = g * 64u + lane;
      bool own = q < n;
      uint32_t id = 0;
      float4 s_o = make_float4(0, 0, 0, 0), s_d = make_float4(0, 0, 0, 0);
      if (own) id = q;
      if (own && !fp.primary_implicit) {
         const uint32_t f = q / fp.n_owned, k = q - f * fp.n_owned;
         const uint32_t pix = fp.owned_pixels ? fp.owned_pixels[k] : k;
         uint32_t px = pix % fp.W, py = pix / fp.W;
         uint32_t rng = sample == 0 ? init_rng(px, py, fp.W, fp.frame_numbers[f]) : __float_as_uint(ps.radf[id].w);
         uint32_t seed = rng;
         float jx = random_float(rng), jy = random_float(rng);
         V3 o, d;
         primary_ray(fp, px, py, jx, jy, o, d);
         s_o = make_float4(o.x, o.y, o.z, __uint_as_float(rng));
         s_d = make_float4(d.x, d.y, d.z, __uint_as_float(seed));
      }
      uint32_t shard = own ? shard_of_run(id >> 6) : 0xffffffffu;
      unsigned long long todo = __ballot(own);
      while (todo) {
         const int leader = __ffsll((long long)todo) - 1;
         const uint32_t s = __shfl(shard, leader);
         const bool mine = own && shard == s;
         uint32_t slot = wave_append(&ctl->q_count[qc_index(0, Q_RAY, s)], mine);
         if (mine) {
            const uint32_t pos = s * ps.shard_cap + slot;
            ps.queue[0][pos] = id;
            if (!fp.primary_implicit) {
               st_rec(rec_quad(ps.set[0], pos, REC_ORIGIN), s_o);
               st_rec(rec_quad(ps.set[0], pos, REC_DIR), s_d);
               st_rec(rec_quad(ps.set[0], pos, REC_THR), make_float4(1.0f, 1.0f, 1.0f, 0.0f));
            }
         }
         todo &= ~__ballot(mine);
      }
   }
}

__device__ __forceinline__ void shade_miss_path(const FrameParams& fp, const PathState& ps, uint32_t pos, uint32_t id, uint32_t bounce) {
   const PathRecs rec = ps.set[bounce & 1];
   const bool implicit = bounce == 0 && fp.primary_implicit;
   float4 ro, rd_implicit = make_float4(0.0f, 0.0f, 0.0f, 0.0f);
   if (implicit)
      primary_state(fp, id, ro, rd_implicit);
   else
      ro = ld_rec(rec_quad(rec, pos, REC_ORIGIN));
   V3 sky_color = v3(0.0f, 0.0f, 0.0f);
   if (fp.furnace) {
      sky_color = v3(1.0f, 1.0f, 1.0f);
   } else if (fp.sky_enabled == 1) {
      const float4 rd = implicit ? rd_implicit : ld_rec(rec_quad(rec, pos, REC_DIR));
      V3 c = sky::integrate_scattering(v3(ro.x, ro.y, ro.z), v3(rd.x, rd.y, rd.z), 999999999.0f, v3(fp.sun_dir[0], fp.sun_dir[1], fp.sun_dir[2]));
      sky_color = v3(fminf(c.x, 1.0f), fminf(c.y, 1.0f), fminf(c.z, 1.0f));
   }
   float4 thr = make_float4(1.0f, 1.0f, 1.0f, 0.0f);
   if (!implicit) thr = ld_rec(rec_quad(rec, pos, REC_THR));
   float4 rad = make_float4(0.0f, 0.0f, 0.0f, 0.0f);
   if (bounce != 0) rad = ld_rec(rec_quad(rec, pos, REC_RAD));
   V3 t = v3(thr.x, thr.y, thr.z) * sky_color;
   st_stream(ps.radf + id, make_float4(rad.x + t.x, rad.y + t.y, rad.z + t.z, ro.w));
}

__global__ __launch_bounds__(kBlock) void k_shade_miss(FrameParams fp, PathState ps, Control* ctl, DeviceStats* stats, uint32_t bounce) {
   const ShardCtx sx = shard_ctx();
   const uint32_t seg = sx.shard * ps.shard_cap;
   const uint2* __restrict__ queue = reinterpret_cast<const uint2*>(ps.queue[4]) + seg;
   const uint32_t count = ctl->q_count[qc_index(bounce, Q_MISS, sx.shard)];
   for (uint32_t i = sx.lb * kBlock + threadIdx.x; i < count; i += sx.nb * kBlock) {
      const uint2 e = ld_stream(queue + i);
      shade_miss_path(fp, ps, seg + e.x, e.y, bounce);
   }
   if (sx.lb == 0 && threadIdx.x == 0 && count) atomicAdd(&stats->misses, (unsigned long long)count);
}

__device__ __forceinline__ V3 pbr_weight(V3 N, V3 V, V3 L, V3 base, float metallic, float roughness) {
   const float PI = 3.14159265359f;
   const V3 H = normalize3(V + L);
   const float a = roughness * roughness, a2 = a * a;
   const float NdotH = fmaxf(dot3(N, H), 0.0f), NdotH2 = NdotH * NdotH;
   float denom = NdotH2 * (a2 - 1.0f) + 1.0f;
   denom = (PI * denom) * denom;
   const float NDF = a2 / denom;
   const float NdotV = fmaxf(dot3(N, V), 0.0f), NdotL = fmaxf(dot3(N, L), 0.0f);
   const float r = roughness + 1.0f, k = (r * r) / 8.0f;
   const float gV = NdotV / (NdotV * (1.0f - k) + k), gL = NdotL / (NdotL * (1.0f - k) + k);
   const float G = gL * gV;
   const float c = fminf(fmaxf(1.0f - fmaxf(dot3(H, V), 0.0f), 0.0f), 1.0f);
   const float c5 = ((c * c) * (c * c)) * c;
   const float om = 1.0f - metallic;
   const V3 F0 = v3(0.04f * om + base.x * metallic, 0.04f * om + base.y * metallic, 0.04f * om + base.z * metallic);
   const V3 F = v3(F0.x + (1.0f - F0.x) * c5, F0.y + (1.0f - F0.y) * c5, F0.z + (1.0f - F0.z) * c5);
   const V3 kD = v3((1.0f - F.x) * om, (1.0f - F.y) * om, (1.0f - F.z) * om);
   const float den = (4.0f * NdotV) * NdotL + 0.0001f;
   const float dg = NDF * G;
   const V3 spec = v3((dg * F.x) / den, (dg * F.y) / den, (dg * F.z) / den);
   return v3(kD.x * base.x + spec.x * PI, kD.y * base.y + spec.y * PI, kD.z * base.z + spec.z * PI);
}

__device__ __forceinline__ float schlick_reflectance(float cosine, float ref_idx) {
   float r0 = (1.0f - ref_idx) / (1.0f + ref_idx);
   r0 = r0 * r0;
   float x = 1.0f - cosine;
   float x5 = ((x * x) * (x * x)) * x;
   return r0 + (1.0f - r0) * x5;
}
__device__ __forceinline__ V3 reflect3(V3 I, V3 N) { return I - N * (2.0f * dot3(N, I)); }
__device__ __forceinline__ V3 refract3(V3 I, V3 N, float eta) {
   float dn = dot3(N, I);
   float k = 1.0f - eta * eta * (1.0f - dn * dn);
   if (k < 0.0f) return v3(0, 0, 0);
   return I * eta - N * (eta * dn + sqrtf(k));
}

struct SurfaceHit {
   V3 world_normal, origin;
   float uu, vv;
   uint32_t mesh_index;
};
__device__ __forceinline__ void surface_normal_uv(const float4 s0, const float4 s1, const float4 s2, const float4 s3, float bu, float bv, V3& normal, float& uu, float& vv) {
   const V3 n0 = v3(s0.x, s0.y, s0.z), n1 = v3(s0.w, s1.x, s1.y), n2 = v3(s1.z, s1.w, s2.x);
   const float uv0x = s2.y, uv0y = s2.z, uv1x = s2.w, uv1y = s3.x, uv2x = s3.y, uv2y = s3.z;
   const float bx = 1.0f - bu - bv, by = bu, bz = bv;
   normal = (n0 * bx + n1 * by) + n2 * bz;
   uu = (uv0x * bx + uv1x * by) + uv2x * bz;
   vv = (uv0y * bx + uv1y * by) + uv2y * bz;
}
__device__ __forceinline__ V3 world_normal_of(const MeshShade& ms, V3 normal, V3 ray_dir) {
   V3 wn = v3((normal.x * ms.w2o[0] + normal.y * ms.w2o[3]) + normal.z * ms.w2o[6],
              (normal.x * ms.w2o[1] + normal.y * ms.w2o[4]) + normal.z * ms.w2o[7],
              (normal.x * ms.w2o[2] + normal.y * ms.w2o[5]) + normal.z * ms.w2o[8]);
   V3 world_normal = normalize3(wn);
   if (dot3(world_normal, ray_dir) > 0.0f) world_normal = vneg(world_normal);
   return world_normal;
}
__device__ __forceinline__ bool path_scatters(const MeshShade& ms, V3 ray_dir, V3 world_normal) {
   return (ms.type == 0.0f || ms.type == 4.0f) ? dot3(ray_dir, world_normal) < 0.0f : (ms.type == 1.0f || ms.type == 2.0f);
}
__device__ __forceinline__ V3 material_scatter(const MeshShade& ms, V3 ray_dir, V3 world_normal, V3& color, uint32_t& seed) {
   V3 scatter = v3(0, 0, 0);
   if (ms.type == 0.0f) {
      scatter = world_normal + random_point_in_unit_sphere(seed);
   } else if (ms.type == 1.0f) {
      scatter = reflect3(normalize3(ray_dir), world_normal);
      scatter = scatter + ms.property * random_point_in_unit_sphere(seed);
      color = v3(1, 1, 1);
   } else if (ms.type == 2.0f) {
      V3 nd = normalize3(ray_dir);
      float dnd = dot3(nd, world_normal);
      V3 outward = dnd > 0 ? vneg(world_normal) : world_normal;
      float ratio = ms.property;
      ratio = dnd > 0 ? ratio : 1.0f / ratio;
      float cos_theta = fminf(dot3(-1.0f * nd, outward), 1.0f);
      float sin_theta = sqrtf(1.0f - cos_theta * cos_theta);
      bool cannot_refract = ratio * sin_theta > 1.0f;
      float reflectance = schlick_reflectance(cos_theta, ratio);
      if (cannot_refract || reflectance > random_float(seed))
         scatter = reflect3(nd, outward);
      else
         scatter = refract3(nd, outward, ratio);
      color = v3(1, 1, 1);
   } else if (ms.type == 4.0f) {
      scatter = world_normal + random_point_in_unit_sphere(seed);
      color = pbr_weight(world_normal, -1.0f * normalize3(ray_dir), normalize3(scatter), color, ms.metallic, ms.roughness);
   } else {
      color = v3(1, 1, 1);
   }
   return scatter;
}
__device__ __forceinline__ bool select_light(const FrameParams& fp, const SceneDev& sc, uint32_t id, uint32_t& rng_x, V3 origin, float& f, int& light_index) {
   float light_sample_weight = 0.0f, total_weights = 1.0f;
   const uint32_t k = id % fp.n_owned;
   const uint32_t pix = fp.owned_pixels ? fp.owned_pixels[k] : k;
   uint32_t px = pix % fp.W;
   bool use_reservoir = (px > fp.W / 2 || fp.full_frame_restir) && fp.use_ris == 1;
   if (use_reservoir) {
      UhReservoir rs = fp.spatial_of[id / fp.n_owned][pix];
      light_sample_weight = rs.W_X;
      total_weights = rs.W_sum;
      light_index = rs.Y;
   } else {
      sample_light_uniform(fp.num_lights_used, rng_x, light_index, light_sample_weight);
      light_sample_weight = 1.0f / light_sample_weight;
   }
   if (total_weights != 0.0f) {
      f = target_function(sc.lights, sc.num_lights, light_index, origin) * light_sample_weight;
      return true;
   }
   return false;
}

__global__ __launch_bounds__(kBlock, kShadeHitBlocks) void k_shade_hit(FrameParams fp, SceneDev sc, PathState ps, Control* ctl, DeviceStats* stats, uint32_t bounce) {
   __shared__ float s_lut[256];
   s_lut[threadIdx.x] = sc.unorm_lut[threadIdx.x];
   constexpr uint32_t kLdsMeshes = 192, kLdsTextures = 64;
   __shared__ MeshShade s_mesh[kLdsMeshes];
   __shared__ TexInfo s_tex[kLdsTextures];
   const uint32_t n_lds_mesh = sc.num_meshes < kLdsMeshes ? sc.num_meshes : kLdsMeshes;
   const uint32_t n_lds_tex = sc.num_textures < kLdsTextures ? sc.num_textures : kLdsTextures;
   __shared__ uint32_t s_hits;
   __shared__ uint32_t s_list[kWavesPerBlock][6][128];
   __shared__ uint32_t s_miss[kWavesPerBlock][2][128];
   if (threadIdx.x == 0) s_hits = 0;
   if (threadIdx.x < n_lds_mesh) s_mesh[threadIdx.x] = sc.meshes[threadIdx.x];
   if (threadIdx.x < n_lds_tex) s_tex[threadIdx.x] = sc.textures[threadIdx.x];
   __syncthreads();
   const ShardCtx sx = shard_ctx();
   const uint32_t seg = sx.shard * ps.shard_cap;
   const uint32_t count = ctl->q_count[qc_index(bounce, Q_RAY, sx.shard)];
   const uint32_t* __restrict__ queue = ps.queue[bounce & 1] + seg;
   const PathRecs cur = ps.set[bounce & 1], nxt = ps.set[(bounce + 1) & 1];
   uint32_t* q_next = ps.queue[(bounce + 1) & 1] + seg;
   uint32_t* n_next = &ctl->q_count[qc_index(bounce + 1, Q_RAY, sx.shard)];
   uint32_t* q_light = ps.queue[2] + seg;
   uint32_t* n_light = &ctl->q_count[qc_index(bounce, Q_LIGHT, sx.shard)];
   uint2* q_miss = reinterpret_cast<uint2*>(ps.queue[4]) + seg;
   uint32_t* n_miss = &ctl->q_count[qc_index(bounce, Q_MISS, sx.shard)];
   const uint32_t stride = sx.nb * kBlock;
   const uint32_t rounds = (count + stride - 1) / stride;
   uint32_t n_hits = 0;
   auto shade = [&](uint32_t id, uint32_t pos, float4 hr, bool valid) {
      const uint32_t pk = __float_as_uint(hr.w);
      bool scattered = false, want_light = false;
      uint32_t slot = 0;
      float4 n_o = make_float4(0, 0, 0, 0), n_d = make_float4(0, 0, 0, 0), n_t = make_float4(0, 0, 0, 0), n_r = make_float4(0, 0, 0, 0);
      if (valid) {
         float4 ro, rd, thr4;
         if (bounce == 0 && fp.primary_implicit) {
            primary_state(fp, id, ro, rd);
            thr4 = make_float4(1.0f, 1.0f, 1.0f, 0.0f);
         } else {
            ro = ld_rec(rec_quad(cur, seg + pos, REC_ORIGIN));
            rd = ld_rec(rec_quad(cur, seg + pos, REC_DIR));
            thr4 = ld_rec(rec_quad(cur, seg + pos, REC_THR));
         }
         uint2 rng = make_uint2(__float_as_uint(ro.w), __float_as_uint(rd.w));
         float4 rad4 = make_float4(0.0f, 0.0f, 0.0f, 0.0f);
         if (bounce != 0) rad4 = ld_rec(rec_quad(cur, seg + pos, REC_RAD));
         const V3 ray_dir = v3(rd.x, rd.y, rd.z);
         const float t = hr.x, bu = hr.y, bv = hr.z;
         const float4* sp = sc.shade + 4 * (size_t)pk;
         float4 s0 = sp[0], s1 = sp[1], s2 = sp[2], s3 = sp[3];
         const uint32_t mesh_index = __float_as_uint(s3.w);
         MeshShade ms = lds_fetch(s_mesh + (mesh_index < kLdsMeshes ? mesh_index : kLdsMeshes - 1));
         if (mesh_index >= n_lds_mesh) ms = sc.meshes[mesh_index];
         V3 normal;
         float uu, vv;
         surface_normal_uv(s0, s1, s2, s3, bu, bv, normal, uu, vv);
         asm volatile("" : "+v"(rng.x), "+v"(rng.y), "+v"(thr4.x), "+v"(thr4.y), "+v"(thr4.z), "+v"(rad4.x), "+v"(rad4.y), "+v"(rad4.z));
         const V3 world_normal = world_normal_of(ms, normal, ray_dir);
         V3 origin = v3(ro.x, ro.y, ro.z) + t * ray_dir;
         origin = offset_ray(origin, world_normal);
         scattered = path_scatters(ms, ray_dir, world_normal);
         const unsigned long long scat_mask = __ballot(scattered);
         const int scat_leader = __ffsll((long long)scat_mask) - 1;
         uint32_t scat_base = 0;
         V3 color = sample_texture_pre(sc, s_lut, ms.diffuse_map, uu, vv, s_tex, n_lds_tex, [&] {
            typedef __attribute__((address_space(1))) uint32_t* global_u32_t;
            global_u32_t counter = (global_u32_t)n_next;
            asm volatile("" : "+v"(counter));
            if (scattered && (int)lane_id() == scat_leader) scat_base = __hip_atomic_fetch_add(counter, (uint32_t)__popcll(scat_mask), __ATOMIC_RELAXED, __HIP_MEMORY_SCOPE_AGENT);
         });
         color = color * v3(ms.base_color[0], ms.base_color[1], ms.base_color[2]);

         uint32_t seed = rng.y;
         const V3 scatter = material_scatter(ms, ray_dir, world_normal, color, seed);
         rng.y = seed;
         if (scat_leader >= 0) slot = (uint32_t)__builtin_amdgcn_readlane((int)scat_base, scat_leader) + __builtin_amdgcn_mbcnt_hi((uint32_t)(scat_mask >> 32), __builtin_amdgcn_mbcnt_lo((uint32_t)scat_mask, 0u));

         V3 thr = v3(thr4.x, thr4.y, thr4.z) * color;
         if (!scattered) {
            st_stream(ps.radf + id, make_float4(rad4.x + thr.x, rad4.y + thr.y, rad4.z + thr.z, __uint_as_float(rng.x)));
         } else {
            float f = 0.0f;
            int light_index = 0;
            if (fp.lights_enabled == 1) want_light = select_light(fp, sc, id, rng.x, origin, f, light_index);
            n_o = make_float4(origin.x, origin.y, origin.z, __uint_as_float(rng.x));
            n_d = make_float4(scatter.x, scatter.y, scatter.z, __uint_as_float(rng.y));
            n_t = make_float4(thr.x, thr.y, thr.z, f);
            n_r = make_float4(rad4.x, rad4.y, rad4.z, __uint_as_float((uint32_t)light_index));
         }
      }
      const uint32_t lslot = wave_append(n_light, want_light);
      if (scattered) {
         st_stream(q_next + slot, id);
         st_rec(rec_quad(nxt, seg + slot, REC_ORIGIN), n_o);
         if (bounce + 1 < fp.num_bounces) st_rec(rec_quad(nxt, seg + slot, REC_DIR), n_d);
         st_rec(rec_quad(nxt, seg + slot, REC_THR), n_t);
         st_rec(rec_quad(nxt, seg + slot, REC_RAD), n_r);
      }
      if (want_light) st_stream(q_light + lslot, slot);
   };
   uint32_t(*list)[128] = s_list[threadIdx.x >> 6];
   uint32_t(*missed)[128] = s_miss[threadIdx.x >> 6];
   const uint32_t lane = lane_id();
   uint32_t n_list = 0, n_missed = 0;
   auto flush_misses = [&](uint32_t n) {
      uint32_t base = 0;
      if (lane == 0) base = atomicAdd(n_miss, n);
      base = __shfl(base, 0);
      if (lane < n) st_stream(q_miss + base + lane, make_uint2(missed[0][lane], missed[1][lane]));
   };
   auto entry = [&](uint32_t k) { return make_float4(__uint_as_float(list[2][k]), __uint_as_float(list[3][k]), __uint_as_float(list[4][k]), __uint_as_float(list[5][k])); };
   for (uint32_t r = 0; r < rounds; r++) {
      const uint32_t i = r * stride + sx.lb * kBlock + threadIdx.x;
      uint32_t id = 0;
      float4 hr = make_float4(0.0f, 0.0f, 0.0f, __uint_as_float(kEmptyRef));
      if (i < count) {
         id = ld_stream(queue + i);
         hr = ld_rec(ps.hit + seg + i);
      }
      const bool is_hit = __float_as_uint(hr.w) != kEmptyRef;
      const unsigned long long mask = __ballot(is_hit);
      const unsigned long long mmask = __ballot(i < count && !is_hit);
      if (mmask) {
         const uint32_t mp = __builtin_amdgcn_mbcnt_hi((uint32_t)(mmask >> 32), __builtin_amdgcn_mbcnt_lo((uint32_t)mmask, 0u));
         if (i < count && !is_hit) {
            missed[0][n_missed + mp] = i;
            missed[1][n_missed + mp] = id;
         }
         n_missed += (uint32_t)__popcll(mmask);
         __builtin_amdgcn_wave_barrier();
         if (n_missed >= 64u) {
            flush_misses(64u);
            const uint32_t rest = n_missed - 64u;
            uint32_t tmp0 = 0, tmp1 = 0;
            if (lane < rest) {
               tmp0 = missed[0][64u + lane];
               tmp1 = missed[1][64u + lane];
            }
            __builtin_amdgcn_wave_barrier();
            if (lane < rest) {
               missed[0][lane] = tmp0;
               missed[1][lane] = tmp1;
            }
            __builtin_amdgcn_wave_barrier();
            n_missed = rest;
         }
      }
      if (mask == 0ull) continue;
      const uint32_t prefix = __builtin_amdgcn_mbcnt_hi((uint32_t)(mask >> 32), __builtin_amdgcn_mbcnt_lo((uint32_t)mask, 0u));
      if (is_hit) {
         list[0][n_list + prefix] = id;
         list[1][n_list + prefix] = i;
         list[2][n_list + prefix] = __float_as_uint(hr.x);
         list[3][n_list + prefix] = __float_as_uint(hr.y);
         list[4][n_list + prefix] = __float_as_uint(hr.z);
         list[5][n_list + prefix] = __float_as_uint(hr.w);
      }
      n_list += (uint32_t)__popcll(mask);
      __builtin_amdgcn_wave_barrier();
      if (n_list >= 64u) {
         shade(list[0][lane], list[1][lane], entry(lane), true);
         n_hits += 64u;
         const uint32_t rest = n_list - 64u;
         uint32_t tmp[6] = {0, 0, 0, 0, 0, 0};
         if (lane < rest)
            for (int k = 0; k < 6; k++) tmp[k] = list[k][64u + lane];
         __builtin_amdgcn_wave_barrier();
         if (lane < rest)
            for (int k = 0; k < 6; k++) list[k][lane] = tmp[k];
         __builtin_amdgcn_wave_barrier();
         n_list = rest;
      }
   }
   if (n_list) {
      shade(lane < n_list ? list[0][lane] : 0u, lane < n_list ? list[1][lane] : 0u, lane < n_list ? entry(lane) : make_float4(0.0f, 0.0f, 0.0f, 0.0f), lane < n_list);
      n_hits += n_list;
   }
   if (n_missed) flush_misses(n_missed);
   if (lane_id() == 0 && n_hits) atomicAdd(&s_hits, n_hits);
   __syncthreads();
   if (threadIdx.x == 0 && s_hits) atomicAdd(&stats->closest_hits, (unsigned long long)s_hits);
}

__global__ __launch_bounds__(kBlock) void k_flush_survivors(FrameParams fp, PathState ps, Control* ctl) {
   const ShardCtx sx = shard_ctx();
   const uint32_t seg = sx.shard * ps.shard_cap, b = fp.num_bounces;
   const uint32_t count = ctl->q_count[qc_index(b, Q_RAY, sx.shard)];
   const uint32_t* __restrict__ queue = ps.queue[b & 1] + seg;
   const PathRecs rec = ps.set[b & 1];
   for (uint32_t i = sx.lb * kBlock + threadIdx.x; i < count; i += sx.nb * kBlock) {
      const uint32_t id = ld_stream(queue + i);
      const float4 rad = ld_rec(rec_quad(rec, seg + i, REC_RAD)), ro = ld_rec(rec_quad(rec, seg + i, REC_ORIGIN));
      st_stream(ps.radf + id, make_float4(rad.x, rad.y, rad.z, ro.w));
   }
}

template <bool COUNT, bool INLINE>
__device__ __forceinline__ int sun_grid_query(const SunGridDev& g, const float4* __restrict__ packets, V3 o, V3 d, uint32_t& n_tris, uint32_t& n_covered) {
   typedef float f4_t __attribute__((ext_vector_type(4)));
   const f4_t* __restrict__ recs = reinterpret_cast<const f4_t*>(g.recs);
   const f4_t* __restrict__ tris = reinterpret_cast<const f4_t*>(packets);
   const uint2* __restrict__ entries = reinterpret_cast<const uint2*>(g.entries);
   const uint4* __restrict__ cells = reinterpret_cast<const uint4*>(g.cell_start);
   const float pu = dot_fma(v3(g.U[0], g.U[1], g.U[2]), o), pv = dot_fma(v3(g.V[0], g.V[1], g.V[2]), o), pw = dot_fma(v3(g.W[0], g.W[1], g.W[2]), o);
   uint32_t cx, cy;
   sun_cell_of(g, pu, pv, cx, cy);
   if (g.coarse) {
      const float cw = g.coarse[(cy >> g.coarse_shift) * g.coarse_nx + (cx >> g.coarse_shift)];
      if (sun_coarse_covered(cw, pw)) {
         if (COUNT) n_covered++;
         return 1;
      }
   }
   const uint32_t cell = cy * g.nx + cx;
   const uint4 cs = cells[cell];
   const uint32_t end = cells[cell + 1].x;
   const float cover = __uint_as_float(cs.y);
   if (pw < cover && cover - pw < kSunCoverReach) {
      if (COUNT) n_covered++;
      return 1;
   }
   if (cx == 0 || cy == 0 || cx + 1 == g.nx || cy + 1 == g.ny || end - cs.x > g.max_walk) return 2;
   if (cs.x >= end) return 0;
   Hit best;
   best.t = 10000.0f;
   best.u = best.v = 0.0f;
   best.idx = kEmptyRef;
   best.key = 0xffffffffu;
   uint32_t e = cs.x;
   if constexpr (INLINE) {
      const f4_t* r = recs + 4 * (size_t)e;
      for (;;) {
         const f4_t na = r[0], nb = r[1], nc = r[2];
         if (nc.z < pw) return 0;
         if (COUNT) n_tris++;
         if (tri_compute<true>(make_float4(na.x, na.y, na.z, na.w), make_float4(nb.x, nb.y, nb.z, nb.w), make_float4(nc.x, nc.y, nc.z, nc.w), 0u, o, d, 0.001f, INFINITY, best)) return 1;
         e++;
         if (e >= end || nc.w < pw) return 0;
         r += 4;
      }
   } else {
      uint2 cur = make_uint2(cs.z, cs.w);
      for (;;) {
         if (__uint_as_float(cur.y) < pw) return 0;
         const f4_t* r = tris + kTriStride16 * (size_t)cur.x;
         const f4_t na = r[0], nb = r[1], nc = r[2];
         e++;
         const uint2 nx = e < end ? entries[e] : make_uint2(0u, 0u);
         if (COUNT) n_tris++;
         if (tri_compute<true>(make_float4(na.x, na.y, na.z, na.w), make_float4(nb.x, nb.y, nb.z, nb.w), make_float4(nc.x, nc.y, nc.z, nc.w), cur.x, o, d, 0.001f, INFINITY, best)) return 1;
         if (e >= end) return 0;
         cur = nx;
      }
   }
}

constexpr int kFusedBlocks = 4;
struct FusedTraceLds {
   uint32_t stack[kWavesPerBlock][kLdsStack][64];
   RayPool<2> pool[kWavesPerBlock];
};
struct FusedShadeLds {
   uint32_t list[kWavesPerBlock][6][128];
   uint32_t miss[kWavesPerBlock][2][128];
};
template <bool COUNT, bool INLINE>
__global__ __launch_bounds__(kBlock, kFusedBlocks) void k_path_fused(SceneDev sc, FrameParams fp, PathState ps, Control* ctl, DeviceStats* stats, SunGridDev g, bool use_grid,
                                                                      bool sun_of_bounce0) {
   constexpr uint32_t kFirst = 1;
   constexpr uint32_t kHasRay = 1u << 31, kSun = 1u << 30, kLight = 1u << 29, kLeftShift = 23, kLeftMask = 63u << kLeftShift, kPosMask = (1u << kLeftShift) - 1u;
   __shared__ float s_lut[256];
   constexpr uint32_t kLdsMeshes = 128, kLdsTextures = 64;
   __shared__ MeshShade s_mesh[kLdsMeshes];
   __shared__ TexInfo s_tex[kLdsTextures];
   __shared__ union {
      FusedTraceLds t;
      FusedShadeLds s;
   } u;
   __shared__ uint32_t s_cursor, s_count[2];
   const uint32_t n_lds_mesh = sc.num_meshes < kLdsMeshes ? sc.num_meshes : kLdsMeshes;
   const uint32_t n_lds_tex = sc.num_textures < kLdsTextures ? sc.num_textures : kLdsTextures;
   s_lut[threadIdx.x] = sc.unorm_lut[threadIdx.x];
   if (threadIdx.x < n_lds_mesh) s_mesh[threadIdx.x] = sc.meshes[threadIdx.x];
   if (threadIdx.x < n_lds_tex) s_tex[threadIdx.x] = sc.textures[threadIdx.x];
   const uint32_t lane = lane_id();
   const uint32_t wave = threadIdx.x >> 6;
   const ShardCtx sx = shard_ctx();
   const uint32_t seg = sx.shard * ps.shard_cap;
   const PathRecs rec = ps.set[kFirst & 1];
   const uint32_t* __restrict__ ids = ps.queue[kFirst & 1] + seg;
   const uint32_t count1 = ctl->q_count[qc_index(kFirst, Q_RAY, sx.shard)];
   const uint32_t per = (((count1 + sx.nb - 1) / sx.nb) + 63u) & ~63u;
   const uint32_t lo = sx.lb * per < count1 ? sx.lb * per : count1, hi = lo + per < count1 ? lo + per : count1;
   uint32_t* lists[2] = {ps.queue[0] + seg + lo, ps.queue[3] + seg + lo};
   const uint4* __restrict__ nodes = sc.nodes;
   const float4* __restrict__ tris = sc.tris;
   const V3 sun_d = v3(fp.sun_dir[0], fp.sun_dir[1], fp.sun_dir[2]);
   uint32_t n_nodes = 0, n_tris = 0, n_snodes = 0, n_stris = 0, n_lnodes = 0, n_ltris = 0, n_covered = 0;
   uint32_t w_rays = 0, w_hits = 0, w_sun = 0, w_sun_tree = 0, w_light = 0, w_miss = 0;
   const uint32_t n_range = hi - lo;
   const uint32_t left1 = (fp.num_bounces - 2u) << kLeftShift;
   for (uint32_t i0 = 0; i0 < n_range; i0 += kBlock) {
      const uint32_t i = i0 + threadIdx.x;
      const bool valid = i < n_range;
      uint32_t e = (lo + i) | kHasRay | left1;
      bool to_tree = false;
      if (valid && sun_of_bounce0) {
         int r = 2;
         if (use_grid) {
            const float4 ro = ld_rec(rec_quad(rec, seg + lo + i, REC_ORIGIN));
            r = sun_grid_query<COUNT, INLINE>(g, tris, v3(ro.x, ro.y, ro.z), sun_d, n_stris, n_covered);
            if (COUNT) n_snodes++;
         }
         if (r == 0) {
            const float4 t4 = ld_rec(rec_quad(rec, seg + lo + i, REC_THR)), r4 = ld_rec(rec_quad(rec, seg + lo + i, REC_RAD));
            st_rec(rec_quad(rec, seg + lo + i, REC_RAD), make_float4(r4.x + t4.x, r4.y + t4.y, r4.z + t4.z, r4.w));
         }
         if (r == 2) e |= kSun;
         to_tree = r == 2 && use_grid;
      }
      if (valid) lists[0][i] = e;
      if (sun_of_bounce0) {
         w_sun += (uint32_t)__popcll(__ballot(valid));
         w_sun_tree += (uint32_t)__popcll(__ballot(to_tree));
      }
   }
   if (threadIdx.x == 0) {
      s_count[0] = n_range;
      s_count[1] = 0;
      s_cursor = 0;
   }
   __syncthreads();

   auto trace_phase = [&](uint32_t which) {
      uint32_t* lds_col = &u.t.stack[wave][0][lane];
      RayPool<2>& pool = u.t.pool[wave];
      RaySource src;
      src.queue = lists[which];
      src.count = s_count[which];
      src.cursor = &s_cursor;
      src.wave_index = src.num_waves = 0;
      auto source_of = [&](int a, uint32_t e) { return (const float4*)rec_quad(rec, seg + (e & kPosMask), a == 0 ? REC_ORIGIN : REC_DIR); };
      Feeder<2> f;
      Trav t;
      t.cur = kEmptyRef;
      t.sp = 0;
      enum : uint32_t { BOUNCE_RAY = 0, SUN_RAY = 1, LIGHT_RAY = 2 };
      uint32_t kind = BOUNCE_RAY, entry = 0, rng_x = 0, mark_nodes = 0, mark_tris = 0;
      V3 thr = v3(0, 0, 0), rad = v3(0, 0, 0), scatter = v3(0, 0, 0);
      float lf = 0.0f;
      uint32_t light_bits = 0;
      bool dirty = false;
      uint32_t spill[kSpillStack];
      auto next_ray = [&]() {
         const float4 o4 = make_float4(t.o.x, t.o.y, t.o.z, 0.0f);
         if (entry & kSun) {
            entry &= ~kSun;
            const ShadowRay s = make_shadow_ray<false>(sc, fp, o4, make_float4(thr.x, thr.y, thr.z, lf), make_float4(rad.x, rad.y, rad.z, 0.0f));
            trav_init(t, s.ro, s.rd, s.ro.w, s.rd.w, s.tlimit);
            kind = SUN_RAY;
         } else if (entry & kLight) {
            entry &= ~kLight;
            const ShadowRay s = make_shadow_ray<true>(sc, fp, o4, make_float4(thr.x, thr.y, thr.z, lf), make_float4(rad.x, rad.y, rad.z, __uint_as_float(light_bits)));
            trav_init(t, s.ro, s.rd, s.ro.w, s.rd.w, s.tlimit);
            kind = LIGHT_RAY;
         } else {
            const uint32_t p = entry & kPosMask;
            if (entry & kHasRay) {
               if (dirty) st_rec(rec_quad(rec, seg + p, REC_RAD), make_float4(rad.x, rad.y, rad.z, __uint_as_float(light_bits)));
               trav_init(t, o4, make_float4(scatter.x, scatter.y, scatter.z, 0.0f), 0.001f, 10000.0f, INFINITY);
               kind = BOUNCE_RAY;
            } else {
               st_stream(ps.radf + ld_stream(ids + p), make_float4(rad.x, rad.y, rad.z, __uint_as_float(rng_x)));
               t.cur = kEmptyRef;
            }
         }
         if (COUNT) {
            mark_nodes = n_nodes;
            mark_tris = n_tris;
         }
      };
      auto take = [&](uint32_t slot) {
         entry = pool.id[slot];
         const float4 ro = pool.v[0][slot], rd = pool.v[1][slot];
         if (entry & (kSun | kLight)) {
            const uint32_t p = entry & kPosMask;
            const float4 t4 = ld_rec(rec_quad(rec, seg + p, REC_THR)), r4 = ld_rec(rec_quad(rec, seg + p, REC_RAD));
            thr = v3(t4.x, t4.y, t4.z);
            lf = t4.w;
            rad = v3(r4.x, r4.y, r4.z);
            light_bits = __float_as_uint(r4.w);
            scatter = v3(rd.x, rd.y, rd.z);
            rng_x = __float_as_uint(ro.w);
            dirty = false;
            t.o = v3(ro.x, ro.y, ro.z);
            next_ray();
         } else {
            trav_init(t, ro, rd, 0.001f, 10000.0f, INFINITY);
            kind = BOUNCE_RAY;
         }
      };
      while (refill_lanes<2>(f, src, pool, t.cur == kEmptyRef, source_of, take)) {
         if (t.cur != kEmptyRef) {
            bool occluded = false;
            bool ended = trav_step<false, COUNT, true>(nodes, tris, t, lds_col, spill, occluded, n_nodes, n_tris);
            const bool blocked = t.best.idx != kEmptyRef && t.best.t <= t.tlimit;
            if (kind != BOUNCE_RAY && blocked) ended = true;
            if (ended) {
               if (kind == BOUNCE_RAY) {
                  st_rec(ps.hit + seg + (entry & kPosMask), make_float4(t.best.t, t.best.u, t.best.v, __uint_as_float(t.best.idx)));
                  t.cur = kEmptyRef;
               } else {
                  if (!blocked) {
                     rad = kind == SUN_RAY ? v3(rad.x + thr.x, rad.y + thr.y, rad.z + thr.z) : v3(rad.x + thr.x * lf, rad.y + thr.y * lf, rad.z + thr.z * lf);
                     dirty = true;
                  }
                  if (COUNT) {
                     const uint32_t dn = n_nodes - mark_nodes, dt = n_tris - mark_tris;
                     n_nodes = mark_nodes;
                     n_tris = mark_tris;
                     if (kind == SUN_RAY) {
                        n_snodes += dn;
                        n_stris += dt;
                     } else {
                        n_lnodes += dn;
                        n_ltris += dt;
                     }
                  }
                  next_ray();
               }
            }
         }
      }
   };

   uint32_t carry_n = 0, carry_pos = 0, carry_id = 0;
   auto shade_phase = [&](uint32_t which) {
      const uint32_t count = s_count[which];
      const uint32_t* __restrict__ cur_list = lists[which];
      uint32_t* nxt_list = lists[which ^ 1];
      uint32_t(*list)[128] = u.s.list[wave];
      uint32_t(*missed)[128] = u.s.miss[wave];
      uint32_t n_list = 0, n_missed = carry_n, n_rays = 0;
      if (lane < carry_n) {
         missed[0][lane] = carry_pos;
         missed[1][lane] = carry_id;
      }
      __builtin_amdgcn_wave_barrier();
      auto shade = [&](uint32_t id, uint32_t pl, float4 hr, bool valid) {
         bool scattered = false, want_light = false, to_tree = false, keep = false;
         uint32_t flags = 0;
         const uint32_t p = pl & kPosMask;
         if (valid) {
            const uint32_t left = (pl & kLeftMask) >> kLeftShift;
            const bool last = left == 0u;
            const uint32_t pk = __float_as_uint(hr.w);
            const float4 ro = ld_rec(rec_quad(rec, seg + p, REC_ORIGIN)), rd = ld_rec(rec_quad(rec, seg + p, REC_DIR)), thr4 = ld_rec(rec_quad(rec, seg + p, REC_THR)),
                         rad4 = ld_rec(rec_quad(rec, seg + p, REC_RAD));
            uint2 rng = make_uint2(__float_as_uint(ro.w), __float_as_uint(rd.w));
            const V3 ray_dir = v3(rd.x, rd.y, rd.z);
            const float4* sp = sc.shade + 4 * (size_t)pk;
            const float4 s0 = sp[0], s1 = sp[1], s2 = sp[2], s3 = sp[3];
            const uint32_t mesh_index = __float_as_uint(s3.w);
            MeshShade ms = lds_fetch(s_mesh + (mesh_index < kLdsMeshes ? mesh_index : kLdsMeshes - 1));
            if (mesh_index >= n_lds_mesh) ms = sc.meshes[mesh_index];
            V3 normal;
            float uu, vv;
            surface_normal_uv(s0, s1, s2, s3, hr.y, hr.z, normal, uu, vv);
            const V3 world_normal = world_normal_of(ms, normal, ray_dir);
            V3 origin = v3(ro.x, ro.y, ro.z) + hr.x * ray_dir;
            origin = offset_ray(origin, world_normal);
            scattered = path_scatters(ms, ray_dir, world_normal);
            V3 color = sample_texture(sc, s_lut, ms.diffuse_map, uu, vv, s_tex, n_lds_tex);
            color = color * v3(ms.base_color[0], ms.base_color[1], ms.base_color[2]);
            uint32_t seed = rng.y;
            const V3 scatter = material_scatter(ms, ray_dir, world_normal, color, seed);
            rng.y = seed;
            const V3 thr = v3(thr4.x, thr4.y, thr4.z) * color;
            V3 rad = v3(rad4.x, rad4.y, rad4.z);
            if (!scattered) {
               st_stream(ps.radf + id, make_float4(rad.x + thr.x, rad.y + thr.y, rad.z + thr.z, __uint_as_float(rng.x)));
            } else {
               float lf = 0.0f;
               int light_index = 0;
               if (fp.lights_enabled == 1) want_light = select_light(fp, sc, id, rng.x, origin, lf, light_index);
               if (fp.sun_shadow_enabled == 1) {
                  int r = use_grid ? sun_grid_query<COUNT, INLINE>(g, tris, origin, sun_d, n_stris, n_covered) : 2;
                  if (COUNT && use_grid) n_snodes++;
                  if (r == 0) rad = v3(rad.x + thr.x, rad.y + thr.y, rad.z + thr.z);
                  if (r == 2) flags |= kSun;
                  to_tree = r == 2 && use_grid;
               }
               if (want_light) flags |= kLight;
               if (!last) flags |= kHasRay | ((left - 1u) << kLeftShift);
               keep = (flags & (kHasRay | kSun | kLight)) != 0u;
               if (!keep) {
                  st_stream(ps.radf + id, make_float4(rad.x, rad.y, rad.z, __uint_as_float(rng.x)));
               } else {
                  st_rec(rec_quad(rec, seg + p, REC_ORIGIN), make_float4(origin.x, origin.y, origin.z, __uint_as_float(rng.x)));
                  st_rec(rec_quad(rec, seg + p, REC_DIR), make_float4(scatter.x, scatter.y, scatter.z, __uint_as_float(rng.y)));
                  st_rec(rec_quad(rec, seg + p, REC_THR), make_float4(thr.x, thr.y, thr.z, lf));
                  st_rec(rec_quad(rec, seg + p, REC_RAD), make_float4(rad.x, rad.y, rad.z, __uint_as_float((uint32_t)light_index)));
               }
            }
         }
         const uint32_t slot = wave_append(&s_count[which ^ 1], keep);
         if (keep) nxt_list[slot] = p | flags;
         if (fp.sun_shadow_enabled == 1) w_sun += (uint32_t)__popcll(__ballot(scattered));
         w_sun_tree += (uint32_t)__popcll(__ballot(to_tree));
         w_light += (uint32_t)__popcll(__ballot(want_light));
      };
      auto flush_misses = [&](uint32_t n) {
         if (lane < n) shade_miss_path(fp, ps, seg + missed[0][lane], missed[1][lane], kFirst);
         w_miss += n;
      };
      auto entry_of = [&](uint32_t k) { return make_float4(__uint_as_float(list[2][k]), __uint_as_float(list[3][k]), __uint_as_float(list[4][k]), __uint_as_float(list[5][k])); };
      const uint32_t rounds = (count + kBlock - 1) / kBlock;
      for (uint32_t r = 0; r < rounds; r++) {
         const uint32_t i = r * kBlock + threadIdx.x;
         uint32_t id = 0, p = 0;
         float4 hr = make_float4(0.0f, 0.0f, 0.0f, __uint_as_float(kEmptyRef));
         bool has_ray = false;
         if (i < count) {
            const uint32_t e = cur_list[i];
            has_ray = (e & kHasRay) != 0u;
            p = e & (kPosMask | kLeftMask);
            if (has_ray) {
               id = ld_stream(ids + (e & kPosMask));
               hr = ld_rec(ps.hit + seg + (e & kPosMask));
            }
         }
         const bool is_hit = __float_as_uint(hr.w) != kEmptyRef;
         const unsigned long long mask = __ballot(is_hit);
         const unsigned long long mmask = __ballot(has_ray && !is_hit);
         n_rays += (uint32_t)__popcll(__ballot(has_ray));
         if (mmask) {
            const uint32_t mp = __builtin_amdgcn_mbcnt_hi((uint32_t)(mmask >> 32), __builtin_amdgcn_mbcnt_lo((uint32_t)mmask, 0u));
            if (has_ray && !is_hit) {
               missed[0][n_missed + mp] = p & kPosMask;
               missed[1][n_missed + mp] = id;
            }
            n_missed += (uint32_t)__popcll(mmask);
            __builtin_amdgcn_wave_barrier();
            if (n_missed >= 64u) {
               flush_misses(64u);
               const uint32_t rest = n_missed - 64u;
               uint32_t tmp0 = 0, tmp1 = 0;
               if (lane < rest) {
                  tmp0 = missed[0][64u + lane];
                  tmp1 = missed[1][64u + lane];
               }
               __builtin_amdgcn_wave_barrier();
               if (lane < rest) {
                  missed[0][lane] = tmp0;
                  missed[1][lane] = tmp1;
               }
               __builtin_amdgcn_wave_barrier();
               n_missed = rest;
            }
         }
         if (mask == 0ull) continue;
         const uint32_t prefix = __builtin_amdgcn_mbcnt_hi((uint32_t)(mask >> 32), __builtin_amdgcn_mbcnt_lo((uint32_t)mask, 0u));
         if (is_hit) {
            list[0][n_list + prefix] = id;
            list[1][n_list + prefix] = p;
            list[2][n_list + prefix] = __float_as_uint(hr.x);
            list[3][n_list + prefix] = __float_as_uint(hr.y);
            list[4][n_list + prefix] = __float_as_uint(hr.z);
            list[5][n_list + prefix] = __float_as_uint(hr.w);
         }
         n_list += (uint32_t)__popcll(mask);
         __builtin_amdgcn_wave_barrier();
         if (n_list >= 64u) {
            shade(list[0][lane], list[1][lane], entry_of(lane), true);
            w_hits += 64u;
            const uint32_t rest = n_list - 64u;
            uint32_t tmp[6] = {0, 0, 0, 0, 0, 0};
            if (lane < rest)
               for (int k = 0; k < 6; k++) tmp[k] = list[k][64u + lane];
            __builtin_amdgcn_wave_barrier();
            if (lane < rest)
               for (int k = 0; k < 6; k++) list[k][lane] = tmp[k];
            __builtin_amdgcn_wave_barrier();
            n_list = rest;
         }
      }
      if (n_list) {
         shade(lane < n_list ? list[0][lane] : 0u, lane < n_list ? list[1][lane] : 0u, lane < n_list ? entry_of(lane) : make_float4(0.0f, 0.0f, 0.0f, 0.0f), lane < n_list);
         w_hits += n_list;
      }
      carry_n = n_missed;
      if (lane < n_missed) {
         carry_pos = missed[0][lane];
         carry_id = missed[1][lane];
      }
      w_rays += n_rays;
   };

   uint32_t which = 0;
#ifdef UH_FUSED_PROFILE
   unsigned long long c_trace = 0, c_wait = 0, c_shade = 0;
#define UH_TICK(acc)                                  \
   {                                                  \
      const unsigned long long now = wall_clock64();  \
      acc += now - c_last;                            \
      c_last = now;                                   \
   }
   unsigned long long c_last = wall_clock64();
#else
#define UH_TICK(acc)
#endif
   for (uint32_t round_no = 0; round_no < kMaxBounces + 2u; round_no++) {
      if (s_count[which] == 0u && s_count[which ^ 1] == 0u) break;
      trace_phase(which);
      UH_TICK(c_trace)
      __syncthreads();
      UH_TICK(c_wait)
      shade_phase(which);
      UH_TICK(c_shade)
      __syncthreads();
      UH_TICK(c_wait)
      if (threadIdx.x == 0) {
         s_count[which] = 0;
         s_cursor = 0;
      }
      which ^= 1;
      __syncthreads();
   }
   if (carry_n) {
      if (lane < carry_n) shade_miss_path(fp, ps, seg + carry_pos, carry_id, kFirst);
      w_miss += carry_n;
   }
   if (lane == 0) {
      if (w_rays) atomicAdd(&stats->rays[UH_RAY_BOUNCE], (unsigned long long)w_rays);
      if (w_hits) atomicAdd(&stats->closest_hits, (unsigned long long)w_hits);
      if (w_sun) atomicAdd(&stats->rays[UH_RAY_SUN_SHADOW], (unsigned long long)w_sun);
      if (w_sun_tree) atomicAdd(&stats->sun_tree_rays, (unsigned long long)w_sun_tree);
      if (w_light) atomicAdd(&stats->rays[UH_RAY_LIGHT_SHADOW], (unsigned long long)w_light);
      if (w_miss) atomicAdd(&stats->misses, (unsigned long long)w_miss);
   }
   if (COUNT) {
      atomicAdd(&stats->nodes_visited, (unsigned long long)n_nodes);
      atomicAdd(&stats->tris_tested, (unsigned long long)n_tris);
      atomicAdd(&stats->shadow_nodes_visited, (unsigned long long)n_snodes);
      atomicAdd(&stats->shadow_tris_tested, (unsigned long long)n_stris);
      atomicAdd(&stats->light_nodes_visited, (unsigned long long)n_lnodes);
      atomicAdd(&stats->light_tris_tested, (unsigned long long)n_ltris);
      atomicAdd(&stats->sun_covered_rays, (unsigned long long)n_covered);
#ifdef UH_FUSED_PROFILE
      if (lane == 0) {
         atomicAdd(&stats->light_nodes_visited, c_trace);
         atomicAdd(&stats->light_tris_tested, c_wait);
         atomicAdd(&stats->sun_covered_rays, c_shade);
      }
#endif
   }
#undef UH_TICK
}

__device__ __forceinline__ uchar4 resolve_color(float4 acc, uint32_t total_samples, uint32_t limit) {
   float denom = (float)min(total_samples, limit);
   V3 c = v3(acc.x / denom, acc.y / denom, acc.z / denom);
   c = v3(linear_to_srgb(c.x), linear_to_srgb(c.y), linear_to_srgb(c.z));
   return make_uchar4((unsigned char)unorm8(c.z), (unsigned char)unorm8(c.y), (unsigned char)unorm8(c.x), 0);
}

__global__ __launch_bounds__(kBlock) void k_finish_sample(FrameParams fp, PathState ps, Images im, uint32_t sample, bool last) {
   for (uint32_t k = blockIdx.x * kBlock + threadIdx.x; k < fp.n_owned; k += gridDim.x * kBlock) {
      const uint32_t pix = fp.owned_pixels ? fp.owned_pixels[k] : k;
      float4 acc = make_float4(0.0f, 0.0f, 0.0f, 0.0f);
      bool acc_loaded = false;
      uint32_t total = fp.total_samples;
      for (uint32_t f = 0; f < fp.batch_frames; f++) {
         const uint32_t id = f * fp.n_owned + k;
         float4 pc = make_float4(0.0f, 0.0f, 0.0f, 0.0f), rad = make_float4(0.0f, 0.0f, 0.0f, 0.0f);
         if (sample != 0) pc = ps.pixcol[id];
         if (fp.num_bounces != 0) rad = ps.radf[id];
         pc = make_float4(pc.x + rad.x, pc.y + rad.y, pc.z + rad.z, 0.0f);
         if (!last) {
            ps.pixcol[id] = pc;
            continue;
         }
         total = fp.total_samples_of[f];
         if (total != fp.samples_per_frame) {
            if (!acc_loaded) acc = im.accumulation[pix];
         } else {
            acc = make_float4(0.0f, 0.0f, 0.0f, 0.0f);
         }
         acc_loaded = true;
         if (total <= fp.accumulation_limit) acc = make_float4(acc.x + pc.x, acc.y + pc.y, acc.z + pc.z, 0.0f);
         acc.w = 0.0f;
      }
      if (!last) continue;
      im.accumulation[pix] = acc;
      im.output[pix] = resolve_color(acc, total, fp.accumulation_limit);
   }
}

__global__ __launch_bounds__(kBlock) void k_resolve(Images im, uint32_t n, uint32_t total_samples, uint32_t limit) {
   for (uint32_t id = blockIdx.x * kBlock + threadIdx.x; id < n; id += gridDim.x * kBlock)
      im.output[id] = resolve_color(im.accumulation[id], total_samples, limit);
}

__global__ __launch_bounds__(kBlock) void k_gbuffer_generate(FrameParams fp, RawRays ps, RowSpans spans) {
   const uint32_t n = spans.total();
   for (uint32_t j = blockIdx.x * kBlock + threadIdx.x; j < n; j += gridDim.x * kBlock) {
      const uint32_t id = spans.pixel_of(j);
      V3 o, d;
      primary_ray(fp, id % fp.W, id / fp.W, 0.5f, 0.5f, o, d);
      ps.ray_o[j] = make_float4(o.x, o.y, o.z, 0.001f);
      ps.ray_d[j] = make_float4(d.x, d.y, d.z, 10000.0f);
   }
}
__global__ __launch_bounds__(kBlock) void k_gbuffer_resolve(FrameParams fp, RawRays ps, Images im, DeviceStats* stats, RowSpans spans, uint32_t counted) {
   const uint32_t n = spans.total();
   for (uint32_t j = blockIdx.x * kBlock + threadIdx.x; j < n; j += gridDim.x * kBlock) {
      const uint32_t id = spans.pixel_of(j);
      float4 h = ps.hit[j];
      if (__float_as_uint(h.w) != kEmptyRef) {
         float4 ro = ps.ray_o[j], rd = ps.ray_d[j];
         V3 p = v3(ro.x, ro.y, ro.z) + h.x * v3(rd.x, rd.y, rd.z);
         im.gbuffer_pos[id] = make_float4(p.x, p.y, p.z, 1.0f);
      } else {
         im.gbuffer_pos[id] = make_float4(1.0f, 1.0f, 1.0f, 0.0f);
      }
   }
   if (blockIdx.x == 0 && threadIdx.x == 0) atomicAdd(&stats->rays[UH_RAY_GBUFFER], (unsigned long long)counted);
}

__device__ __forceinline__ V3 gbuffer_fetch(const float4* __restrict__ g, uint32_t W, uint32_t px, uint32_t py) {
   uint32_t x0 = px == 0 ? 0 : px - 1, y0 = py == 0 ? 0 : py - 1;
   float4 a = g[(size_t)y0 * W + x0], b = g[(size_t)y0 * W + px], c = g[(size_t)py * W + x0], d = g[(size_t)py * W + px];
   return ((xyz(a) + xyz(b)) + (xyz(c) + xyz(d))) * 0.25f;
}

constexpr uint32_t kMaxLdsLights = UH_MAX_GPU_LIGHTS;

__device__ __forceinline__ void stage_lights(float4* s_lights, const SceneDev& sc) {
   for (uint32_t i = threadIdx.x; i < 2 * sc.num_lights; i += blockDim.x) s_lights[i] = sc.lights[i];
   __syncthreads();
}

__global__ __launch_bounds__(kBlock) void k_reset_reservoirs(Images im, RowSpans spans) {
   const uint32_t n = spans.total();
   for (uint32_t j = blockIdx.x * kBlock + threadIdx.x; j < n; j += gridDim.x * kBlock) {
      const uint32_t id = spans.pixel_of(j);
      UhReservoir z = {-1, 0.0f, 0.0f, 0};
      im.reservoirs[0][id] = z;
      im.reservoirs[1][id] = z;
   }
}

__global__ __launch_bounds__(kBlock) void k_initial_ris(FrameParams fp, SceneDev sc, Images im, RowSpans spans) {
   __shared__ float4 s_lights[2 * kMaxLdsLights];
   stage_lights(s_lights, sc);
   const uint32_t work = spans.total();
   for (uint32_t j = blockIdx.x * kBlock + threadIdx.x; j < work; j += gridDim.x * kBlock) {
      const uint32_t id = spans.pixel_of(j);
      uint32_t px = id % fp.W, py = id / fp.W;
      uint32_t rng = init_rng(px, py, fp.W, fp.frame_number);
      V3 hit_position = gbuffer_fetch(im.gbuffer_pos, fp.W, px, py);
      UhReservoir r = {-1, 0.0f, 0.0f, 0};
      for (int i = 0; i < 32; i++) {
         int cand;
         float p;
         sample_light_uniform(fp.num_lights_used, rng, cand, p);
         float m_i = 1.0f / 32.0f;
         float p_hat = target_function(s_lights, sc.num_lights, cand, hit_position);
         float W_Xi = 1.0f / p;
         float w_i = m_i * p_hat * W_Xi;
         update_reservoir(rng, r, cand, w_i, 1);
      }
      r.M = 1;
      if (r.Y != -1) finalize_resampling(r, target_function(s_lights, sc.num_lights, r.Y, hit_position));
      UhReservoir nr = {-1, 0.0f, 0.0f, 0};
      update_reservoir(rng, nr, r.Y, r.W_sum * (float)r.M, r.M);
      finalize_resampling(nr, target_function(s_lights, sc.num_lights, nr.Y, hit_position));
      im.reservoirs[0][id] = nr;
   }
}

__global__ __launch_bounds__(kBlock) void k_temporal_reuse(FrameParams fp, SceneDev sc, Images im, RowSpans spans) {
   __shared__ float4 s_lights[2 * kMaxLdsLights];
// ... 20 lines not shown
      uy = 1.0f - uy;
      if (ux >= 0.0f && ux <= 1.0f && uy >= 0.0f && uy <= 1.0f) {
         int ix = (int)(ux * (float)fp.W + 0.5f), iy = (int)(uy * (float)fp.H + 0.5f);
         uint32_t ti = (uint32_t)iy * fp.W + (uint32_t)ix;
         if (ti > n - 1) ti = n - 1;
         pr = im.prev_spatial[ti];
      }
      p_hat = pr.Y == -1 ? 0.0f : target_function(s_lights, sc.num_lights, pr.Y, hit_position);
      pr.M = min(20 * ir.M, pr.M);
      update_reservoir(rng, nr, pr.Y, p_hat * pr.W_X * (float)pr.M, pr.M);
      if (nr.Y != -1) finalize_resampling(nr, target_function(s_lights, sc.num_lights, nr.Y, hit_position));
      im.reservoirs[1][id] = nr;
   }
}

__global__ __launch_bounds__(kBlock) void k_spatial_reuse(FrameParams fp, SceneDev sc, Images im, RowSpans spans) {
   __shared__ float4 s_lights[2 * kMaxLdsLights];
   stage_lights(s_lights, sc);
   const uint32_t work = spans.total();
   const UhReservoir* __restrict__ temporal = im.reservoirs[1];
   for (uint32_t j = blockIdx.x * kBlock + threadIdx.x; j < work; j += gridDim.x * kBlock) {
      const uint32_t id = spans.pixel_of(j);
      if (fp.spatial_enabled == 0) {
         im.reservoirs[2][id] = temporal[id];
         continue;
      }
      uint32_t px = id % fp.W, py = id / fp.W;
      uint32_t rng = init_rng(px, py, fp.W, fp.frame_number);
      V3 hit_position = gbuffer_fetch(im.gbuffer_pos, fp.W, px, py);
      UhReservoir nr = {-1, 0.0f, 0.0f, 0};
      UhReservoir tr = temporal[id];
      float p_hat = target_function(s_lights, sc.num_lights, tr.Y, hit_position);
      update_reservoir(rng, nr, tr.Y, p_hat * tr.W_X * (float)tr.M, tr.M);
      for (int i = 0; i < 5; i++) {
         float ox = random_float(rng) * 2.0f - 1.0f, oy = random_float(rng) * 2.0f - 1.0f;
         ox *= 30.0f;
         oy *= 30.0f;
         uint32_t nx = px + (uint32_t)(int)ox, ny = py + (uint32_t)(int)oy;
         nx = min(nx, fp.W - 1);
         ny = min(ny, fp.H - 1);
         UhReservoir nb = temporal[(size_t)ny * fp.W + nx];
         float ph = target_function(s_lights, sc.num_lights, nb.Y, hit_position);
         update_reservoir(rng, nr, nb.Y, ph * nb.W_X * (float)nb.M, nb.M);
      }
      if (nr.Y != -1) finalize_resampling(nr, target_function(s_lights, sc.num_lights, nr.Y, hit_position));
      im.reservoirs[2][id] = nr;
   }
}

template <bool PACK>
__global__ __launch_bounds__(kBlock) void k_tiles(float4* acc, float4* packed, uint32_t W, uint32_t H, uint32_t rank, uint32_t world, uint32_t tile) {
   const uint32_t tiles_x = (W + tile - 1) / tile, tiles_y = (H + tile - 1) / tile;
   const uint32_t num_tiles = tiles_x * tiles_y;
   const uint32_t owned = num_tiles > rank ? (num_tiles - rank + world - 1) / world : 0;
   const uint64_t total = (uint64_t)owned * tile * tile;
   for (uint64_t i = (uint64_t)blockIdx.x * kBlock + threadIdx.x; i < total; i += (uint64_t)gridDim.x * kBlock) {
      uint32_t local = (uint32_t)(i / (tile * tile)), within = (uint32_t)(i % (tile * tile));
      uint32_t t = rank + local * world;
      uint32_t x = (t % tiles_x) * tile + within % tile, y = (t / tiles_x) * tile + within / tile;
      bool inside = x < W && y < H;
      if (PACK)
         packed[i] = inside ? acc[(size_t)y * W + x] : make_float4(0, 0, 0, 0);
      else if (inside)
         acc[(size_t)y * W + x] = packed[i];
   }
}

static inline dim3 stream_grid(const LaunchCfg& c, uint32_t n) {
   uint32_t blocks = (n + kBlock - 1) / kBlock;
   uint32_t cap = c.num_cus * 8;
   return dim3(blocks < cap ? (blocks ? blocks : 1) : cap);
}
static inline dim3 sharded_grid(uint32_t blocks) {
   uint32_t g = (blocks / kShards) * kShards;
   return dim3(g < kShards ? kShards : g);
}
static inline dim3 closest_grid(const LaunchCfg& c) { return sharded_grid(c.num_cus * c.closest_blocks_per_cu); }
static inline dim3 shadow_grid(const LaunchCfg& c) { return sharded_grid(c.num_cus * c.shadow_blocks_per_cu); }
static inline dim3 shade_grid(const LaunchCfg& c, uint32_t n) {
   uint32_t blocks = (n + kBlock - 1) / kBlock, cap = c.num_cus * 8;
   return sharded_grid(blocks < cap ? blocks : cap);
}

uint32_t query_trace_occupancy() {
   int a = 0, b = 0;
   if (hipOccupancyMaxActiveBlocksPerMultiprocessor(&a, k_trace_closest<false>, kBlock, 0) != hipSuccess) a = 4;
   if (hipOccupancyMaxActiveBlocksPerMultiprocessor(&b, k_trace_shadow<false, false>, kBlock, 0) != hipSuccess) b = 4;
   int m = a < b ? a : b;
   if (m < 1) m = 1;
   if (m > 8) m = 8;
   return (uint32_t)m;
}

void launch_generate(const LaunchCfg& c, const FrameParams& fp, const PathState& ps, Control* ctl, uint32_t sample) {
   k_generate<<<stream_grid(c, fp.n_owned * fp.batch_frames), kBlock, 0, c.stream>>>(fp, ps, ctl, sample);
}

static void launch_closest(const LaunchCfg& c, dim3 grid, const SceneDev& sc, bool sharded, const float4* ray_o, const float4* ray_d, float4* hit,
                           uint32_t shard_cap, Control* ctl, DeviceStats* stats, uint32_t bounce, uint32_t cursor_slot, int ray_kind, uint32_t n,
                           const uint32_t* listed = nullptr) {
   if (c.count_visits && sharded)
      k_trace_closest<true><<<grid, kBlock, 0, c.stream>>>(sc, sharded, ray_o, ray_d, hit, shard_cap, ctl, stats, bounce, cursor_slot, ray_kind, n, listed);
   else
      k_trace_closest<false><<<grid, kBlock, 0, c.stream>>>(sc, sharded, ray_o, ray_d, hit, shard_cap, ctl, stats, bounce, cursor_slot, ray_kind, n, listed);
}

void launch_trace_closest(const LaunchCfg& c, const SceneDev& sc, const PathState& ps, Control* ctl, DeviceStats* stats, uint32_t bounce,
                          uint32_t cursor_slot, int ray_kind) {
   const PathRecs& rec = ps.set[bounce & 1];
   launch_closest(c, closest_grid(c), sc, true, rec_quad(rec, 0, REC_ORIGIN), rec_quad(rec, 0, REC_DIR), ps.hit, ps.shard_cap, ctl, stats, bounce, cursor_slot, ray_kind, 0);
}

void launch_trace_camera_grid(const LaunchCfg& c, const FrameParams& fp, const SceneDev& sc, const PathState& ps, Control* ctl, DeviceStats* stats, uint32_t cursor_slot_grid,
                              uint32_t cursor_slot_tree, const SunGridDev& g, bool leftovers_possible) {
   const dim3 grid = sharded_grid(c.num_cus * 8);
   if (c.count_visits)
      k_trace_camera_grid<true><<<grid, kBlock, 0, c.stream>>>(sc, fp, ps, ctl, stats, cursor_slot_grid, g);
   else
      k_trace_camera_grid<false><<<grid, kBlock, 0, c.stream>>>(sc, fp, ps, ctl, stats, cursor_slot_grid, g);
   if (!leftovers_possible) return;
   const PathRecs& rec = ps.set[0];
   launch_closest(c, closest_grid(c), sc, true, rec_quad(rec, 0, REC_ORIGIN), rec_quad(rec, 0, REC_DIR), ps.hit, ps.shard_cap, ctl, stats, 0, cursor_slot_tree, UH_RAY_PRIMARY, 0, ps.queue[3]);
}

void launch_shade_miss(const LaunchCfg& c, const FrameParams& fp, const PathState& ps, Control* ctl, DeviceStats* stats, uint32_t bounce) {
   const dim3 full = shade_grid(c, fp.n_owned * fp.batch_frames), lean = sharded_grid(c.num_cus * 8);
   k_shade_miss<<<full.x < lean.x ? full : lean, kBlock, 0, c.stream>>>(fp, ps, ctl, stats, bounce);
}

void launch_shade_hit(const LaunchCfg& c, const FrameParams& fp, const SceneDev& sc, const PathState& ps, const Images& im, Control* ctl,
                      DeviceStats* stats, uint32_t bounce) {
   k_shade_hit<<<shade_grid(c, fp.W * fp.H), kBlock, 0, c.stream>>>(fp, sc, ps, ctl, stats, bounce);
}
void launch_flush_survivors(const LaunchCfg& c, const FrameParams& fp, const PathState& ps, Control* ctl) {
   k_flush_survivors<<<shade_grid(c, fp.n_owned * fp.batch_frames), kBlock, 0, c.stream>>>(fp, ps, ctl);
}

void launch_path_fused(const LaunchCfg& c, const FrameParams& fp, const SceneDev& sc, const PathState& ps, Control* ctl, DeviceStats* stats, const SunGridDev& g,
                       bool use_grid, bool sun_of_bounce0) {
   const dim3 grid = sharded_grid(c.num_cus * c.fused_blocks_per_cu);
#define UH_FUSED(COUNT, INLINE) k_path_fused<COUNT, INLINE><<<grid, kBlock, 0, c.stream>>>(sc, fp, ps, ctl, stats, g, use_grid, sun_of_bounce0)
   if (use_grid && g.recs) {
      if (c.count_visits) UH_FUSED(true, true);
      else UH_FUSED(false, true);
   } else {
      if (c.count_visits) UH_FUSED(true, false);
      else UH_FUSED(false, false);
   }
#undef UH_FUSED
}

void launch_trace_shadow(const LaunchCfg& c, const FrameParams& fp, const SceneDev& sc, const PathState& ps, Control* ctl, DeviceStats* stats,
                         uint32_t bounce, uint32_t cursor_slot, bool light, bool sun_leftovers) {
#define UH_SHADOW(COUNT, LIGHT) k_trace_shadow<COUNT, LIGHT><<<shadow_grid(c), kBlock, 0, c.stream>>>(sc, fp, ps, ctl, stats, bounce, cursor_slot, sun_leftovers)
   if (light) {
      if (c.count_visits) UH_SHADOW(true, true);
      else UH_SHADOW(false, true);
   } else {
      if (c.count_visits) UH_SHADOW(true, false);
      else UH_SHADOW(false, false);
   }
#undef UH_SHADOW
}

void launch_trace_sun_grid(const LaunchCfg& c, const FrameParams& fp, const SceneDev& sc, const PathState& ps, Control* ctl, DeviceStats* stats, uint32_t bounce,
                           uint32_t cursor_slot, const SunGridDev& g) {
   const dim3 grid = sharded_grid(c.num_cus * 8);
#define UH_SUN_GRID(COUNT, INLINE) k_trace_sun_grid<COUNT, INLINE><<<grid, kBlock, 0, c.stream>>>(sc, fp, ps, ctl, stats, bounce, cursor_slot, g)
   if (g.recs) {
      if (c.count_visits) UH_SUN_GRID(true, true);
      else UH_SUN_GRID(false, true);
   } else {
      if (c.count_visits) UH_SUN_GRID(true, false);
      else UH_SUN_GRID(false, false);
   }
#undef UH_SUN_GRID
}

void launch_finish_sample(const LaunchCfg& c, const FrameParams& fp, const PathState& ps, const Images& im, uint32_t sample, bool last) {
   k_finish_sample<<<stream_grid(c, fp.n_owned), kBlock, 0, c.stream>>>(fp, ps, im, sample, last);
}

void launch_resolve(const LaunchCfg& c, const Images& im, uint32_t W, uint32_t H, uint32_t total_samples, uint32_t limit) {
   k_resolve<<<stream_grid(c, W * H), kBlock, 0, c.stream>>>(im, W * H, total_samples, limit);
}

void launch_gbuffer(const LaunchCfg& c, const FrameParams& fp, const SceneDev& sc, const RawRays& ps, const Images& im, DeviceStats* stats, const RowSpans& spans, uint32_t counted,
                    const SunGridDev* camera_grid) {
   const uint32_t n = spans.total();
   if (n == 0) return;
   k_gbuffer_generate<<<stream_grid(c, n), kBlock, 0, c.stream>>>(fp, ps, spans);
   if (camera_grid)
      k_gbuffer_camera_grid<<<stream_grid(c, n), kBlock, 0, c.stream>>>(sc, ps, spans, fp.W, *camera_grid);
   else {
      const uint32_t full = c.num_cus * c.closest_blocks_per_cu, need = (n + kBlock - 1) / kBlock;
      launch_closest(c, dim3(need < full ? need : full), sc, false, ps.ray_o, ps.ray_d, ps.hit, 0, nullptr, stats, 0, 0, 0, n);
   }
   k_gbuffer_resolve<<<stream_grid(c, n), kBlock, 0, c.stream>>>(fp, ps, im, stats, spans, counted);
}

static inline dim3 reservoir_grid(const LaunchCfg& c, const RowSpans& spans) {
   const uint32_t full = c.num_cus * 4, need = (spans.total() + kBlock - 1) / kBlock;
   return dim3(need < full ? (need ? need : 1) : full);
}
void launch_reset_reservoirs(const LaunchCfg& c, const FrameParams& fp, const Images& im, const RowSpans& spans) {
   if (spans.total()) k_reset_reservoirs<<<stream_grid(c, spans.total()), kBlock, 0, c.stream>>>(im, spans);
}
void launch_initial_ris(const LaunchCfg& c, const FrameParams& fp, const SceneDev& sc, const Images& im, const RowSpans& spans) {
   if (spans.total()) k_initial_ris<<<reservoir_grid(c, spans), kBlock, 0, c.stream>>>(fp, sc, im, spans);
}
void launch_temporal_reuse(const LaunchCfg& c, const FrameParams& fp, const SceneDev& sc, const Images& im, const RowSpans& spans) {
   if (spans.total()) k_temporal_reuse<<<reservoir_grid(c, spans), kBlock, 0, c.stream>>>(fp, sc, im, spans);
}
void launch_spatial_reuse(const LaunchCfg& c, const FrameParams& fp, const SceneDev& sc, const Images& im, const RowSpans& spans) {
   if (spans.total()) k_spatial_reuse<<<reservoir_grid(c, spans), kBlock, 0, c.stream>>>(fp, sc, im, spans);
}

void launch_trace_closest_raw(const LaunchCfg& c, const SceneDev& sc, const float4* ray_o, const float4* ray_d, float4* hit, uint32_t n) {
   const uint32_t full = c.num_cus * c.closest_blocks_per_cu, need = (n + kBlock - 1) / kBlock;
   launch_closest(c, dim3(need < full ? (need ? need : 1) : full), sc, false, ray_o, ray_d, hit, 0, nullptr, nullptr, 0, 0, 0, n);
}
void launch_trace_any_raw(const LaunchCfg& c, const SceneDev& sc, const float4* ray_o, const float4* ray_d, uint32_t* occluded, uint32_t n) {
   k_trace_any_raw<<<stream_grid(c, n), kBlock, 0, c.stream>>>(sc, ray_o, ray_d, occluded, n);
}

__global__ __launch_bounds__(kBlock) void k_compose_tiles(Images im, const float4* __restrict__ all, uint64_t stride, uint32_t W, uint32_t H, uint32_t rank, uint32_t world,
                                                           uint32_t tile, uint32_t total_samples, uint32_t limit) {
   const uint32_t tiles_x = (W + tile - 1) / tile, n = W * H;
   for (uint32_t pix = blockIdx.x * kBlock + threadIdx.x; pix < n; pix += gridDim.x * kBlock) {
      const uint32_t x = pix % W, y = pix / W;
      const uint32_t t = (y / tile) * tiles_x + x / tile, owner = t % world;
      float4 acc;
      if (owner == rank)
         acc = im.accumulation[pix];
      else {
         acc = all[owner * stride + (uint64_t)(t / world) * tile * tile + (y % tile) * tile + x % tile];
         im.accumulation[pix] = acc;
      }
      im.output[pix] = resolve_color(acc, total_samples, limit);
   }
}
void launch_compose_tiles(const LaunchCfg& c, const Images& im, const float4* all, uint64_t stride, uint32_t W, uint32_t H, uint32_t rank, uint32_t world, uint32_t tile,
                          uint32_t total_samples, uint32_t limit) {
   k_compose_tiles<<<stream_grid(c, W * H), kBlock, 0, c.stream>>>(im, all, stride, W, H, rank, world, tile, total_samples, limit);
}

void launch_pack_tiles(const LaunchCfg& c, const float4* acc, float4* out, uint32_t W, uint32_t H, uint32_t rank, uint32_t world, uint32_t tile) {
   k_tiles<true><<<stream_grid(c, W * H), kBlock, 0, c.stream>>>(const_cast<float4*>(acc), out, W, H, rank, world, tile);
}
void launch_unpack_tiles(const LaunchCfg& c, float4* acc, const float4* in, uint32_t W, uint32_t H, uint32_t rank, uint32_t world, uint32_t tile) {
   k_tiles<false><<<stream_grid(c, W * H), kBlock, 0, c.stream>>>(acc, const_cast<float4*>(in), W, H, rank, world, tile);
}

__global__ __launch_bounds__(kBlock) void k_hybrid_clear(HybridDev hd, uint32_t n) {
   for (uint32_t i = blockIdx.x * kBlock + threadIdx.x; i < n; i += gridDim.x * kBlock) {
      const float4 one = make_float4(1.0f, 1.0f, 1.0f, 0.0f);
      hd.pos[i] = one;
      hd.nrm[i] = one;
      hd.pbr[i] = one;
      hd.alb[i] = make_uchar4(255, 255, 255, 0);
      hd.shadow[i] = 255;
      hd.refl[i] = make_uchar4(255, 255, 255, 0);
   }
}

__global__ __launch_bounds__(kBlock) void k_hybrid_gbuffer_resolve(SceneDev sc, HybridDev hd, uint32_t n) {
   for (uint32_t j = blockIdx.x * kBlock + threadIdx.x; j < n; j += gridDim.x * kBlock) {
      const float4 h = hd.pos[j], ro = hd.nrm[j], rd = hd.pbr[j];
      const uint32_t packet = __float_as_uint(h.w);
      const float4 clear = make_float4(1.0f, 1.0f, 1.0f, 0.0f);
      float4 pos = clear, nrm = clear, pbr = clear;
      uchar4 alb = make_uchar4(255, 255, 255, 0);
      if (packet != kEmptyRef) {
         const V3 p = v3(ro.x, ro.y, ro.z) + h.x * v3(rd.x, rd.y, rd.z);
         pos = make_float4(p.x, p.y, p.z, 1.0f);
         const uint32_t key = __float_as_uint(sc.tris[kTriStride16 * (size_t)packet + 2].y);
         const uint32_t mesh = key >> kPrimBits, prim = key & kPrimMask;
         const HybridMesh m = hd.meshes[mesh];
         const uint32_t* tri = hd.indices + m.index_base + 3 * (size_t)prim;
         const UhVertex* vb = hd.vertices + m.vertex_base;
         const UhVertex& v0 = vb[tri[0]];
         const UhVertex& v1 = vb[tri[1]];
         const UhVertex& v2 = vb[tri[2]];
         const float b0 = 1.0f - h.y - h.z, b1 = h.y, b2 = h.z;
         V3 nn;
         float uu, vv;
         surface_attributes(sc, m, v0, v1, v2, b0, b1, b2, nn, uu, vv);
         gbuffer_targets(sc, m, mesh, nn, uu, vv, nrm, alb, pbr);
      }
      hd.pos[j] = pos;
      hd.nrm[j] = nrm;
      hd.alb[j] = alb;
      hd.pbr[j] = pbr;
   }
}

__global__ __launch_bounds__(kBlock, 5) void k_hybrid_shadow(SceneDev sc, HybridDev hd) {
   __shared__ uint32_t s_stack[kWavesPerBlock][kLdsStack][64];
   __shared__ RayPool<0> s_pool[kWavesPerBlock];
   const uint32_t lane = lane_id();
   const uint32_t wave = threadIdx.x >> 6;
   uint32_t* lds_col = &s_stack[wave][0][lane];
   RayPool<0>& pool = s_pool[wave];
   RaySource src;
   src.queue = nullptr;
   src.count = hd.W * hd.H;
   src.cursor = nullptr;
   src.wave_index = blockIdx.x * kWavesPerBlock + wave;
   src.num_waves = gridDim.x * kWavesPerBlock;
   auto source_of = [](int, uint32_t) { return (const float4*)nullptr; };
   Feeder<0> f;
   Trav t;
   t.cur = kEmptyRef;
   t.sp = 0;
   uint32_t pix = 0, n_nodes = 0, n_tris = 0;
   uint32_t spill[kSpillStack];
   const V3 sun = v3(hd.sun_dir[0], hd.sun_dir[1], hd.sun_dir[2]);
   auto take = [&](uint32_t slot) {
      pix = f.pool_base + slot;
      const uint32_t px = pix % hd.W, py = pix / hd.W;
      const V3 p = gbuffer_fetch(hd.pos, hd.W, px, py), nn = gbuffer_fetch(hd.nrm, hd.W, px, py);
      const V3 o = offset_ray(p, nn);
      trav_init(t, make_float4(o.x, o.y, o.z, 0.001f), make_float4(sun.x, sun.y, sun.z, 10000.0f), 0.001f, 10000.0f, INFINITY);
   };
   while (refill_lanes<0>(f, src, pool, t.cur == kEmptyRef, source_of, take)) {
      if (t.cur != kEmptyRef) {
         bool occluded = false;
// ... 403 lines not shown
```

Before: 9922.

## Record sun-shadow verdicts as a bitmask and apply them during shading

Sun-shadow kernels (grid and leftover tree walk) now write one lit bit per path into a per-slot bitmask instead of reading throughput and radiance and writing radiance back. The following shade, miss and finish kernels read the bit and add the sun contribution themselves. The bounce-1 radiance record is no longer stored because it is zero. This removes float4 read-modify-write traffic in the shadow pass, at the cost of an extra bitmask read, atomicOr in the leftover kernel, and packing a flag into the high bit of queue positions. It only applies when the sun grid is used, point lights are off, and the fused path is not taken.

```diff
diff --git a/rust-renderer_amd/csrc/context.hip b/rust-renderer_amd/csrc/context.hip
--- a/rust-renderer_amd/csrc/context.hip
+++ b/rust-renderer_amd/csrc/context.hip
@@ -87,6 +87,7 @@
    hipEvent_t frame_start = nullptr, frame_stop = nullptr;
    DevBuf<float4> rec, radf, pixcol;
    DevBuf<uint32_t> queues[5];
+   DevBuf<unsigned long long> sun_lit;
    DevBuf<Control> control;
    PathState ps{};
    bool ready = false;
@@ -101,6 +102,7 @@
          for (uint32_t r = 0; r < runs; r++) per_shard[shard_of_run(r)]++;
          for (uint32_t s = 0; s < kShards; s++) shard_cap = per_shard[s] * 64 > shard_cap ? per_shard[s] * 64 : shard_cap;
       }
+      if (shard_cap >= (1u << 31)) return hipErrorInvalidValue;
       hipError_t e;
 #define SLOT_TRY(expr)                 \
    if ((e = (expr)) != hipSuccess) return e
@@ -116,6 +118,8 @@
       SLOT_TRY(radf.alloc(n, 1 * stagger));
       SLOT_TRY(pixcol.alloc(n, 2 * stagger));
       for (int qi = 0; qi < 5; qi++) SLOT_TRY(queues[qi].alloc((size_t)shard_cap * kShards * (qi == 4 ? 2 : 1)));
+      SLOT_TRY(sun_lit.alloc((size_t)shard_cap * kShards / 64));
+      SLOT_TRY(hipMemsetAsync(sun_lit.p, 0, sun_lit.n * sizeof(unsigned long long), stream));
       SLOT_TRY(control.alloc(1));
       SLOT_TRY(hipMemsetAsync(control.p, 0, sizeof(Control), stream));
       SLOT_TRY(hipStreamSynchronize(stream));
@@ -126,6 +130,7 @@
       ps.radf = radf.p;
       ps.pixcol = pixcol.p;
       for (int i = 0; i < 5; i++) ps.queue[i] = queues[i].p;
+      ps.sun_lit = sun_lit.p;
       ps.shard_cap = shard_cap;
       ready = true;
       return hipSuccess;
@@ -137,6 +142,7 @@
       radf.release();
       pixcol.release();
       for (auto& q : queues) q.release();
+      sun_lit.release();
       control.release();
       for (hipEvent_t* ev : {&ev_traced, &ev_missed, &ev_shaded, &ev_shadowed, &ev_side_done, &ev_acc, &frame_start, &frame_stop}) {
          if (*ev) (void)hipEventDestroy(*ev);
@@ -237,6 +243,7 @@
    uint32_t bvh_nodes = 0, bvh_tris = 0;
 
    bool sun_grid_enabled = true;
+   bool sun_verdicts = true;
    bool sun_valid = false;
    bool sun_attempted = false;
    bool sun_have_pending = false;
@@ -1378,7 +1385,8 @@
    return UH_OK;
 }
 
-static int enqueue_path_trace(uh_ctx* c, Slot& s, const FrameParams& fp) {
+static int enqueue_path_trace(uh_ctx* c, Slot& s, const FrameParams& frame) {
+   FrameParams fp = frame;
    LaunchCfg lc = cfg(c);
    lc.stream = s.stream;
    if (fp.batch_frames == 1) {
@@ -1395,6 +1403,7 @@
       const bool fused = c->fused_bounces && fp.batch_frames == 1 && fp.num_bounces >= 2 && fp.num_bounces <= 64 && s.ps.shard_cap < (1u << 23) &&
                          ((gpu_idle && fp.n_owned <= uh_ctx::kFusedMaxPaths) || c->fused_always);
       const bool fused_sun0 = fused && fp.sun_shadow_enabled == 1 && fp.lights_enabled != 1;
+      fp.sun_verdicts = (c->sun_verdicts && c->sun_this_frame && fp.sun_shadow_enabled == 1 && fp.lights_enabled != 1 && !fused) ? 1u : 0u;
       for (uint32_t b = 0; b < (fused ? 1u : fp.num_bounces); b++) {
          begin_timed(c, (b == 0 && c->cam_this_frame) ? 3 : 0, s.stream);
          if (b == 0 && c->cam_this_frame) {
@@ -1993,7 +2002,9 @@
       if (!range(-1, 1 << 20)) return bad("must be -1 (auto: 4 x the packet array), 0 (off) .. 1048576");
       c->sun_inline_max_mb = value;
       c->sun_attempted = false;
-   } else if (n == "sun_grid_coarse") {
+   } else if (n == "sun_verdicts")
+      c->sun_verdicts = value != 0;
+   else if (n == "sun_grid_coarse") {
       if (!range(0, 6)) return bad("(log2 of the block edge in cells) must be 0..6");
       c->sun_coarse_shift = (uint32_t)value;
       c->sun_attempted = false;
diff --git a/rust-renderer_amd/csrc/device_types.h b/rust-renderer_amd/csrc/device_types.h
--- a/rust-renderer_amd/csrc/device_types.h
+++ b/rust-renderer_amd/csrc/device_types.h
@@ -83,6 +83,7 @@
    uint32_t samples_per_frame, total_samples, num_bounces, accumulation_limit;
    uint32_t sky_enabled, sun_shadow_enabled, lights_enabled, use_ris, full_frame_restir;
    uint32_t primary_implicit;
+   uint32_t sun_verdicts;
    uint32_t furnace;
    uint32_t num_lights_used;
    uint32_t temporal_enabled, spatial_enabled;
@@ -103,6 +104,7 @@
    float4* radf;
    float4* pixcol;
    uint32_t* queue[5];
+   unsigned long long* sun_lit;
    uint32_t shard_cap;
 };
 __host__ __device__ inline float4* rec_quad(const PathRecs& rec, uint32_t pos, int quad) { return rec.base + rec.plane * (size_t)quad + pos; }
diff --git a/rust-renderer_amd/csrc/kernels.hip b/rust-renderer_amd/csrc/kernels.hip
--- a/rust-renderer_amd/csrc/kernels.hip
+++ b/rust-renderer_amd/csrc/kernels.hip
@@ -433,40 +433,50 @@
 }
 
 struct ShadowRay {
-   float4 ro, rd, lit;
+   float4 ro, rd;
    float tlimit;
 };
 template <bool LIGHT>
-__device__ __forceinline__ ShadowRay make_shadow_ray(const SceneDev& sc, const FrameParams& fp, float4 ro, float4 thr, float4 rad) {
+__device__ __forceinline__ ShadowRay make_shadow_ray(const SceneDev& sc, const FrameParams& fp, float4 ro, uint32_t light_bits) {
    ShadowRay s;
    s.ro = make_float4(ro.x, ro.y, ro.z, 0.001f);
    s.tlimit = INFINITY;
    if (LIGHT) {
-      const int light_index = (int)__float_as_uint(rad.w);
+      const int light_index = (int)light_bits;
       V3 lpos = v3(0, 0, 0);
       if (light_index >= 0 && (uint32_t)light_index < sc.num_lights) lpos = xyz(sc.lights[2 * light_index]);
       const V3 o = v3(ro.x, ro.y, ro.z);
       const V3 dir = normalize3(lpos - o);
       s.tlimit = length3(lpos - o);
-      const float f = thr.w;
-      s.lit = make_float4(rad.x + thr.x * f, rad.y + thr.y * f, rad.z + thr.z * f, rad.w);
       s.rd = make_float4(dir.x, dir.y, dir.z, 10000.0f);
    } else {
-      s.lit = make_float4(rad.x + thr.x, rad.y + thr.y, rad.z + thr.z, rad.w);
       s.rd = make_float4(fp.sun_dir[0], fp.sun_dir[1], fp.sun_dir[2], 10000.0f);
    }
    return s;
 }
-
-template <bool COUNT, bool LIGHT>
+template <bool LIGHT>
+__device__ __forceinline__ float4 shadow_lit(float4 thr, float4 rad) {
+   if (LIGHT) {
+      const float f = thr.w;
+      return make_float4(rad.x + thr.x * f, rad.y + thr.y * f, rad.z + thr.z * f, rad.w);
+   }
+   return make_float4(rad.x + thr.x, rad.y + thr.y, rad.z + thr.z, rad.w);
+}
+__device__ __forceinline__ unsigned long long* sun_lit_word(const PathState& ps, uint32_t pos) { return ps.sun_lit + (pos >> 6); }
+__device__ __forceinline__ bool rad_stored(const FrameParams& fp, uint32_t b) { return b > fp.sun_verdicts; }
+constexpr uint32_t kSunLitBit = 0x80000000u;
+
+template <bool COUNT, bool LIGHT, bool VERDICT = false>
 __global__ __launch_bounds__(kBlock, 5) void k_trace_shadow(SceneDev sc, FrameParams fp, PathState ps, Control* ctl, DeviceStats* stats, uint32_t bounce,
                                                               uint32_t cursor_slot, bool leftovers) {
    __shared__ uint32_t s_stack[kWavesPerBlock][kLdsStack][64];
-   __shared__ RayPool<3> s_pool[kWavesPerBlock];
+   static_assert(!(VERDICT && LIGHT), "verdicts are the sun rays'");
+   constexpr int NA = VERDICT ? 1 : 3;
+   __shared__ RayPool<NA> s_pool[kWavesPerBlock];
    const uint32_t lane = lane_id();
    const uint32_t wave = threadIdx.x >> 6;
    uint32_t* lds_col = &s_stack[wave][0][lane];
-   RayPool<3>& pool = s_pool[wave];
+   RayPool<NA>& pool = s_pool[wave];
    const ShardCtx sx = shard_ctx();
    const uint32_t seg = sx.shard * ps.shard_cap;
    RaySource src;
@@ -483,7 +493,7 @@
    const PathRecs rec = ps.set[(bounce + 1) & 1];
    float4* rad = rec_quad(rec, seg, REC_RAD);
    auto source_of = [&](int a, uint32_t pos) { return (const float4*)rec_quad(rec, seg + pos, a == 0 ? REC_ORIGIN : a == 1 ? REC_THR : REC_RAD); };
-   Feeder<3> f;
+   Feeder<NA> f;
    Trav t;
    t.cur = kEmptyRef;
    t.sp = 0;
@@ -492,14 +502,25 @@
    uint32_t spill[kSpillStack];
    auto take = [&](uint32_t slot) {
       id = pool.id[slot];
-      const ShadowRay s = make_shadow_ray<LIGHT>(sc, fp, pool.v[0][slot], pool.v[1][slot], pool.v[2][slot]);
-      lit = s.lit;
+      ShadowRay s;
+      if constexpr (VERDICT) {
+         s = make_shadow_ray<false>(sc, fp, pool.v[0][slot], 0u);
+      } else {
+         const float4 thr = pool.v[1][slot], r4 = pool.v[2][slot];
+         s = make_shadow_ray<LIGHT>(sc, fp, pool.v[0][slot], __float_as_uint(r4.w));
+         lit = shadow_lit<LIGHT>(thr, r4);
+      }
       trav_init(t, s.ro, s.rd, s.ro.w, s.rd.w, s.tlimit);
    };
-   while (refill_lanes<3>(f, src, pool, t.cur == kEmptyRef, source_of, take)) {
+   while (refill_lanes<NA>(f, src, pool, t.cur == kEmptyRef, source_of, take)) {
       if (t.cur != kEmptyRef) {
          bool occluded = false;
-         if (trav_step<true, COUNT>(nodes, tris, t, lds_col, spill, occluded, n_nodes, n_tris) && !occluded) st_stream(rad + id, lit);
+         if (trav_step<true, COUNT>(nodes, tris, t, lds_col, spill, occluded, n_nodes, n_tris) && !occluded) {
+            if constexpr (VERDICT)
+               atomicOr(sun_lit_word(ps, seg + id), 1ull << (id & 63u));
+            else
+               st_stream(rad + id, lit);
+         }
       }
    }
    if (COUNT) {
@@ -528,7 +549,7 @@
 }
 __device__ __forceinline__ bool sun_coarse_covered(float coarse, float pw) { return pw < coarse && coarse - pw < kSunCoarseReach; }
 
-template <bool COUNT, bool INLINE>
+template <bool COUNT, bool INLINE, bool VERDICT>
 __global__ __launch_bounds__(kBlock) void k_trace_sun_grid(SceneDev sc, FrameParams fp, PathState ps, Control* ctl, DeviceStats* stats, uint32_t bounce,
                                                             uint32_t cursor_slot, SunGridDev g) {
    const uint32_t lane = lane_id();
@@ -683,18 +704,26 @@
             lit[k] = !occluded;
          }
       });
-      float4 thr[K], rad[K];
-      static_for<K>([&](auto kc) {
-         constexpr int k = decltype(kc)::value;
-         if (lit[k]) {
-            thr[k] = ld_rec(rec_quad(rec, seg + id[k], REC_THR));
-            rad[k] = ld_rec(rec_quad(rec, seg + id[k], REC_RAD));
-         }
-      });
-      static_for<K>([&](auto kc) {
-         constexpr int k = decltype(kc)::value;
-         if (lit[k]) st_rec(rec_quad(rec, seg + id[k], REC_RAD), make_float4(rad[k].x + thr[k].x, rad[k].y + thr[k].y, rad[k].z + thr[k].z, rad[k].w));
-      });
+      if constexpr (VERDICT) {
+         static_for<K>([&](auto kc) {
+            constexpr int k = decltype(kc)::value;
+            const unsigned long long word = __ballot(lit[k]);
+            if (lane == 0 && base + 64u * k < count) *sun_lit_word(ps, seg + base + 64u * k) = word;
+         });
+      } else {
+         float4 thr[K], rad[K];
+         static_for<K>([&](auto kc) {
+            constexpr int k = decltype(kc)::value;
+            if (lit[k]) {
+               thr[k] = ld_rec(rec_quad(rec, seg + id[k], REC_THR));
+               rad[k] = ld_rec(rec_quad(rec, seg + id[k], REC_RAD));
+            }
+         });
+         static_for<K>([&](auto kc) {
+            constexpr int k = decltype(kc)::value;
+            if (lit[k]) st_rec(rec_quad(rec, seg + id[k], REC_RAD), shadow_lit<false>(thr[k], rad[k]));
+         });
+      }
       static_for<K>([&](auto kc) {
          constexpr int k = decltype(kc)::value;
          if (__ballot(defer[k]) != 0ull) {
@@ -870,7 +899,7 @@
    }
 }
 
-__device__ __forceinline__ void shade_miss_path(const FrameParams& fp, const PathState& ps, uint32_t pos, uint32_t id, uint32_t bounce) {
+__device__ __forceinline__ void shade_miss_path(const FrameParams& fp, const PathState& ps, uint32_t pos, uint32_t id, uint32_t bounce, bool sun_lit) {
    const PathRecs rec = ps.set[bounce & 1];
    const bool implicit = bounce == 0 && fp.primary_implicit;
    float4 ro, rd_implicit = make_float4(0.0f, 0.0f, 0.0f, 0.0f);
@@ -889,7 +918,8 @@
    float4 thr = make_float4(1.0f, 1.0f, 1.0f, 0.0f);
    if (!implicit) thr = ld_rec(rec_quad(rec, pos, REC_THR));
    float4 rad = make_float4(0.0f, 0.0f, 0.0f, 0.0f);
-   if (bounce != 0) rad = ld_rec(rec_quad(rec, pos, REC_RAD));
+   if (rad_stored(fp, bounce)) rad = ld_rec(rec_quad(rec, pos, REC_RAD));
+   if (sun_lit) rad = shadow_lit<false>(thr, rad);
    V3 t = v3(thr.x, thr.y, thr.z) * sky_color;
    st_stream(ps.radf + id, make_float4(rad.x + t.x, rad.y + t.y, rad.z + t.z, ro.w));
 }
@@ -901,7 +931,7 @@
    const uint32_t count = ctl->q_count[qc_index(bounce, Q_MISS, sx.shard)];
    for (uint32_t i = sx.lb * kBlock + threadIdx.x; i < count; i += sx.nb * kBlock) {
       const uint2 e = ld_stream(queue + i);
-      shade_miss_path(fp, ps, seg + e.x, e.y, bounce);
+      shade_miss_path(fp, ps, seg + (e.x & ~kSunLitBit), e.y, bounce, (e.x & kSunLitBit) != 0u);
    }
    if (sx.lb == 0 && threadIdx.x == 0 && count) atomicAdd(&stats->misses, (unsigned long long)count);
 }
@@ -1051,7 +1081,9 @@
    const uint32_t stride = sx.nb * kBlock;
    const uint32_t rounds = (count + stride - 1) / stride;
    uint32_t n_hits = 0;
-   auto shade = [&](uint32_t id, uint32_t pos, float4 hr, bool valid) {
+   auto shade = [&](uint32_t id, uint32_t pos_lit, float4 hr, bool valid) {
+      const uint32_t pos = pos_lit & ~kSunLitBit;
+      const bool sun_lit = (pos_lit & kSunLitBit) != 0u;
       const uint32_t pk = __float_as_uint(hr.w);
       bool scattered = false, want_light = false;
       uint32_t slot = 0;
@@ -1068,7 +1100,7 @@
          }
          uint2 rng = make_uint2(__float_as_uint(ro.w), __float_as_uint(rd.w));
          float4 rad4 = make_float4(0.0f, 0.0f, 0.0f, 0.0f);
-         if (bounce != 0) rad4 = ld_rec(rec_quad(cur, seg + pos, REC_RAD));
+         if (rad_stored(fp, bounce)) rad4 = ld_rec(rec_quad(cur, seg + pos, REC_RAD));
          const V3 ray_dir = v3(rd.x, rd.y, rd.z);
          const float t = hr.x, bu = hr.y, bv = hr.z;
          const float4* sp = sc.shade + 4 * (size_t)pk;
@@ -1080,6 +1112,7 @@
          float uu, vv;
          surface_normal_uv(s0, s1, s2, s3, bu, bv, normal, uu, vv);
          asm volatile("" : "+v"(rng.x), "+v"(rng.y), "+v"(thr4.x), "+v"(thr4.y), "+v"(thr4.z), "+v"(rad4.x), "+v"(rad4.y), "+v"(rad4.z));
+         if (sun_lit) rad4 = shadow_lit<false>(thr4, rad4);
          const V3 world_normal = world_normal_of(ms, normal, ray_dir);
          V3 origin = v3(ro.x, ro.y, ro.z) + t * ray_dir;
          origin = offset_ray(origin, world_normal);
@@ -1119,7 +1152,7 @@
          st_rec(rec_quad(nxt, seg + slot, REC_ORIGIN), n_o);
          if (bounce + 1 < fp.num_bounces) st_rec(rec_quad(nxt, seg + slot, REC_DIR), n_d);
          st_rec(rec_quad(nxt, seg + slot, REC_THR), n_t);
-         st_rec(rec_quad(nxt, seg + slot, REC_RAD), n_r);
+         if (rad_stored(fp, bounce + 1)) st_rec(rec_quad(nxt, seg + slot, REC_RAD), n_r);
       }
       if (want_light) st_stream(q_light + lslot, slot);
    };
@@ -1127,6 +1160,7 @@
    uint32_t(*missed)[128] = s_miss[threadIdx.x >> 6];
    const uint32_t lane = lane_id();
    uint32_t n_list = 0, n_missed = 0;
+   const bool verdicts = bounce != 0 && fp.sun_verdicts != 0;
    auto flush_misses = [&](uint32_t n) {
       uint32_t base = 0;
       if (lane == 0) base = atomicAdd(n_miss, n);
@@ -1142,13 +1176,18 @@
          id = ld_stream(queue + i);
          hr = ld_rec(ps.hit + seg + i);
       }
+      uint32_t i_lit = i;
+      if (verdicts) {
+         const uint32_t i0 = __builtin_amdgcn_readfirstlane(i - lane);
+         if (i0 < count && ((*sun_lit_word(ps, seg + i0) >> lane) & 1ull)) i_lit |= kSunLitBit;
+      }
       const bool is_hit = __float_as_uint(hr.w) != kEmptyRef;
       const unsigned long long mask = __ballot(is_hit);
       const unsigned long long mmask = __ballot(i < count && !is_hit);
       if (mmask) {
          const uint32_t mp = __builtin_amdgcn_mbcnt_hi((uint32_t)(mmask >> 32), __builtin_amdgcn_mbcnt_lo((uint32_t)mmask, 0u));
          if (i < count && !is_hit) {
-            missed[0][n_missed + mp] = i;
+            missed[0][n_missed + mp] = i_lit;
             missed[1][n_missed + mp] = id;
          }
          n_missed += (uint32_t)__popcll(mmask);
@@ -1174,7 +1213,7 @@
       const uint32_t prefix = __builtin_amdgcn_mbcnt_hi((uint32_t)(mask >> 32), __builtin_amdgcn_mbcnt_lo((uint32_t)mask, 0u));
       if (is_hit) {
          list[0][n_list + prefix] = id;
-         list[1][n_list + prefix] = i;
+         list[1][n_list + prefix] = i_lit;
          list[2][n_list + prefix] = __float_as_uint(hr.x);
          list[3][n_list + prefix] = __float_as_uint(hr.y);
          list[4][n_list + prefix] = __float_as_uint(hr.z);
@@ -1214,7 +1253,13 @@
    const PathRecs rec = ps.set[b & 1];
    for (uint32_t i = sx.lb * kBlock + threadIdx.x; i < count; i += sx.nb * kBlock) {
       const uint32_t id = ld_stream(queue + i);
-      const float4 rad = ld_rec(rec_quad(rec, seg + i, REC_RAD)), ro = ld_rec(rec_quad(rec, seg + i, REC_ORIGIN));
+      float4 rad = make_float4(0.0f, 0.0f, 0.0f, 0.0f);
+      if (rad_stored(fp, b)) rad = ld_rec(rec_quad(rec, seg + i, REC_RAD));
+      const float4 ro = ld_rec(rec_quad(rec, seg + i, REC_ORIGIN));
+      if (fp.sun_verdicts) {
+         const uint32_t i0 = __builtin_amdgcn_readfirstlane(i - lane_id());
+         if ((*sun_lit_word(ps, seg + i0) >> lane_id()) & 1ull) rad = shadow_lit<false>(ld_rec(rec_quad(rec, seg + i, REC_THR)), rad);
+      }
       st_stream(ps.radf + id, make_float4(rad.x, rad.y, rad.z, ro.w));
    }
 }
@@ -1380,12 +1425,12 @@
          const float4 o4 = make_float4(t.o.x, t.o.y, t.o.z, 0.0f);
          if (entry & kSun) {
             entry &= ~kSun;
-            const ShadowRay s = make_shadow_ray<false>(sc, fp, o4, make_float4(thr.x, thr.y, thr.z, lf), make_float4(rad.x, rad.y, rad.z, 0.0f));
+            const ShadowRay s = make_shadow_ray<false>(sc, fp, o4, 0u);
             trav_init(t, s.ro, s.rd, s.ro.w, s.rd.w, s.tlimit);
             kind = SUN_RAY;
          } else if (entry & kLight) {
             entry &= ~kLight;
-            const ShadowRay s = make_shadow_ray<true>(sc, fp, o4, make_float4(thr.x, thr.y, thr.z, lf), make_float4(rad.x, rad.y, rad.z, __uint_as_float(light_bits)));
+            const ShadowRay s = make_shadow_ray<true>(sc, fp, o4, light_bits);
             trav_init(t, s.ro, s.rd, s.ro.w, s.rd.w, s.tlimit);
             kind = LIGHT_RAY;
          } else {
@@ -1535,7 +1580,7 @@
          w_light += (uint32_t)__popcll(__ballot(want_light));
       };
       auto flush_misses = [&](uint32_t n) {
-         if (lane < n) shade_miss_path(fp, ps, seg + missed[0][lane], missed[1][lane], kFirst);
+         if (lane < n) shade_miss_path(fp, ps, seg + missed[0][lane], missed[1][lane], kFirst, false);
          w_miss += n;
       };
       auto entry_of = [&](uint32_t k) { return make_float4(__uint_as_float(list[2][k]), __uint_as_float(list[3][k]), __uint_as_float(list[4][k]), __uint_as_float(list[5][k])); };
@@ -1652,7 +1697,7 @@
       __syncthreads();
    }
    if (carry_n) {
-      if (lane < carry_n) shade_miss_path(fp, ps, seg + carry_pos, carry_id, kFirst);
+      if (lane < carry_n) shade_miss_path(fp, ps, seg + carry_pos, carry_id, kFirst, false);
       w_miss += carry_n;
    }
    if (lane == 0) {
@@ -1979,13 +2024,17 @@
 
 void launch_trace_shadow(const LaunchCfg& c, const FrameParams& fp, const SceneDev& sc, const PathState& ps, Control* ctl, DeviceStats* stats,
                          uint32_t bounce, uint32_t cursor_slot, bool light, bool sun_leftovers) {
-#define UH_SHADOW(COUNT, LIGHT) k_trace_shadow<COUNT, LIGHT><<<shadow_grid(c), kBlock, 0, c.stream>>>(sc, fp, ps, ctl, stats, bounce, cursor_slot, sun_leftovers)
-   if (light) {
-      if (c.count_visits) UH_SHADOW(true, true);
-      else UH_SHADOW(false, true);
+#define UH_SHADOW(COUNT, LIGHT, VERDICT) \
+   k_trace_shadow<COUNT, LIGHT, VERDICT><<<shadow_grid(c), kBlock, 0, c.stream>>>(sc, fp, ps, ctl, stats, bounce, cursor_slot, sun_leftovers)
+   if (!light && sun_leftovers && fp.sun_verdicts) {
+      if (c.count_visits) UH_SHADOW(true, false, true);
+      else UH_SHADOW(false, false, true);
+   } else if (light) {
+      if (c.count_visits) UH_SHADOW(true, true, false);
+      else UH_SHADOW(false, true, false);
    } else {
-      if (c.count_visits) UH_SHADOW(true, false);
-      else UH_SHADOW(false, false);
+      if (c.count_visits) UH_SHADOW(true, false, false);
+      else UH_SHADOW(false, false, false);
    }
 #undef UH_SHADOW
 }
@@ -1993,13 +2042,15 @@
 void launch_trace_sun_grid(const LaunchCfg& c, const FrameParams& fp, const SceneDev& sc, const PathState& ps, Control* ctl, DeviceStats* stats, uint32_t bounce,
                            uint32_t cursor_slot, const SunGridDev& g) {
    const dim3 grid = sharded_grid(c.num_cus * 8);
-#define UH_SUN_GRID(COUNT, INLINE) k_trace_sun_grid<COUNT, INLINE><<<grid, kBlock, 0, c.stream>>>(sc, fp, ps, ctl, stats, bounce, cursor_slot, g)
+#define UH_SUN_GRID(COUNT, INLINE)                                                                                                      \
+   if (fp.sun_verdicts) k_trace_sun_grid<COUNT, INLINE, true><<<grid, kBlock, 0, c.stream>>>(sc, fp, ps, ctl, stats, bounce, cursor_slot, g); \
+   else k_trace_sun_grid<COUNT, INLINE, false><<<grid, kBlock, 0, c.stream>>>(sc, fp, ps, ctl, stats, bounce, cursor_slot, g)
    if (g.recs) {
-      if (c.count_visits) UH_SUN_GRID(true, true);
-      else UH_SUN_GRID(false, true);
+      if (c.count_visits) { UH_SUN_GRID(true, true); }
+      else { UH_SUN_GRID(false, true); }
    } else {
-      if (c.count_visits) UH_SUN_GRID(true, false);
-      else UH_SUN_GRID(false, false);
+      if (c.count_visits) { UH_SUN_GRID(true, false); }
+      else { UH_SUN_GRID(false, false); }
    }
 #undef UH_SUN_GRID
 }
```

New measurement: 10220 (median of 6 runs). 1.03x the previous value.
